# osmr/pytorchcv

Measured on AMD Instinct MI355X. Metric: images/sec @224x224 (resnet50 bs=256/GPU), higher is better.
Workload: dtype bf16; 1 GPU; resnet50_bs256; per_gpu_batch=256, global_batch=256, input=fp32 NCHW 224x224 resident in HBM, parallelism=batch-sharded replicas x1, launcher_choice=timed at capture on this GPU

## Files before the change

include/pcv_amd.h:

```cpp
#ifndef PCV_AMD_H
#define PCV_AMD_H

#include <stddef.h>
#include <stdint.h>

#ifdef __cplusplus
extern "C" {
#endif

#define PCV_ABI_VERSION 5

typedef struct pcv_ctx pcv_ctx;

typedef enum pcv_status {
    PCV_OK = 0,
    PCV_ERR_INVALID = -1,
    PCV_ERR_HIP = -2,
    PCV_ERR_NO_DEVICE = -3,
    PCV_ERR_TOO_LARGE = -4
} pcv_status;

typedef enum pcv_dtype { PCV_F32 = 0, PCV_BF16 = 1, PCV_F16 = 2 } pcv_dtype;

typedef enum pcv_act {
// ... 30 lines not shown
int pcv_fp16_guard_begin(pcv_ctx* ctx, unsigned* slot, void* stream);
int pcv_fp16_guard_end(pcv_ctx* ctx, const unsigned* slot, float* y, long count, void* stream);
int pcv_fp16_overflow_count(pcv_ctx* ctx, unsigned* count, void* stream);

int pcv_nchw_to_nhwc(pcv_ctx* ctx, const float* x, void* y, int N, int C, int H, int W,
                     int cpitch, int wpitch, int dtype, void* stream);
int pcv_nhwc_to_nchw(pcv_ctx* ctx, const void* x, float* y, int N, int C, int H, int W, int cpitch, int dtype,
                     void* stream);

int pcv_preprocess_u8(pcv_ctx* ctx, const unsigned char* x, void* y, int N, int Hs, int Ws, int C, int top, int left,
                      int H, int W, int wpitch, const float* mean, const float* inv_std, int dtype, void* stream);

int pcv_conv_packed_bytes(const pcv_conv_desc* d, size_t* bytes);
int pcv_conv_pack(pcv_ctx* ctx, const pcv_conv_desc* d, const float* w, void* packed, void* stream);
int pcv_dwconv_packed_bytes(const pcv_conv_desc* d, size_t* bytes);
int pcv_dwconv_pack(pcv_ctx* ctx, const pcv_conv_desc* d, const float* w, void* packed, void* stream);
int pcv_bn_fold(pcv_ctx* ctx, int C, const float* gamma, const float* beta, const float* mean, const float* var,
                float eps, const float* conv_bias, float* scale, float* shift, void* stream);

int pcv_conv2d_fused(pcv_ctx* ctx, const pcv_conv_desc* d, const void* x, const void* packed,
                     const float* scale, const float* shift, const void* residual, void* y, void* stream);

int pcv_conv2d_gated_fused(pcv_ctx* ctx, const pcv_conv_desc* d, const void* x, const void* packed, const float* scale,
                           const float* shift, const float* gate, const void* residual, void* y, void* stream);
int pcv_fc_f32(pcv_ctx* ctx, const float* in, const float* w, const float* b, float* out, int N, int K, int J, int act,
               void* stream);
int pcv_conv2d_maxpool_supported(const pcv_conv_desc* d, int k, int s, int p, int ceil_mode);
int pcv_conv2d_maxpool_fused(pcv_ctx* ctx, const pcv_conv_desc* d, const void* x, const void* packed, const float* scale,
                             const float* shift, void* y, int k, int s, int p, int ceil_mode, void* stream);

int pcv_conv2d_nchw_stem_supported(const pcv_conv_desc* d, int pool);
int pcv_conv2d_nchw_stem_fused(pcv_ctx* ctx, const pcv_conv_desc* d, const float* x_nchw, const void* packed, const float* scale,
                               const float* shift, void* y, int pool, void* stream);
int pcv_dwconv2d_fused(pcv_ctx* ctx, const pcv_conv_desc* d, const void* x, const void* packed,
                       const float* scale, const float* shift, const void* residual, void* y, void* stream);
int pcv_maxpool2d(pcv_ctx* ctx, const void* x, void* y, int N, int H, int W, int C, int k, int s, int p,
                  int ceil_mode, int dtype, void* stream);
int pcv_channel_slice(pcv_ctx* ctx, const void* x, void* y, long rows, int C, int offset, int x_cpitch, int y_cpitch,
                      int dtype, void* stream);
int pcv_channel_interleave2(pcv_ctx* ctx, const void* a, const void* b, void* y, long rows, int Ch, int a_cpitch,
                            int b_cpitch, int y_cpitch, int dtype, void* stream);
int pcv_channel_concat(pcv_ctx* ctx, const void* x, void* y, long rows, int C, int x_cpitch, int y_cpitch, int y_offset,
                       int dtype, void* stream);
int pcv_interpolate(pcv_ctx* ctx, const void* x, void* y, int N, int H, int W, int C, int Ho, int Wo, int bilinear,
                    int align_corners, int dtype, void* stream);
int pcv_avgpool2d(pcv_ctx* ctx, const void* x, void* y, int N, int H, int W, int C, int k, int s,
                  int dtype, int out_dtype, void* stream);
int pcv_global_avgpool(pcv_ctx* ctx, const void* x, void* y, int N, int HW, int C, int dtype, int out_dtype,
                       void* stream);
int pcv_gemm_bias(pcv_ctx* ctx, const void* x, const void* packed, const float* bias, void* y,
                  int N, int Cin, int Cout, int dtype, int out_dtype, void* stream);
int pcv_se_squeeze(pcv_ctx* ctx, const void* x, float* mean, int N, int HW, int C, int dtype, void* stream);
int pcv_se_excite(pcv_ctx* ctx, const float* mean, const float* w1, const float* b1, const float* w2,
                  const float* b2, float* mid, float* gate, int N, int C, int M, int mid_act, int out_act,
                  void* stream);
int pcv_se_scale(pcv_ctx* ctx, const void* x, const float* gate, const void* residual, void* y,
                 int N, int HW, int C, int post_act, int dtype, void* stream);

int pcv_splat_squeeze(pcv_ctx* ctx, const void* x, float* s, int N, int HW, int C, int radix, int dtype, void* stream);
int pcv_splat_excite(pcv_ctx* ctx, const float* s, const float* w1, const float* b1, const float* w2, const float* b2, float* mid,
                     float* logits, float* att, int N, int C, int M, int radix, int groups, void* stream);
int pcv_splat_combine(pcv_ctx* ctx, const void* x, const float* att, const void* residual, void* y, int N, int HW, int C, int radix,
                      int post_act, int dtype, void* stream);
int pcv_avgpool2d_pad(pcv_ctx* ctx, const void* x, void* y, int N, int H, int W, int C, int k, int s, int p, int ceil_mode,
                      int count_include_pad, int dtype, int out_dtype, void* stream);

int pcv_conv1x1_pair_supported(const pcv_conv_desc* d1, const pcv_conv_desc* d2);
int pcv_conv1x1_pair_fused(pcv_ctx* ctx, const pcv_conv_desc* d1, const pcv_conv_desc* d2, const void* x,
                           const void* packed1, const float* scale1, const float* shift1, const void* residual, void* y1,
                           const void* packed2, const float* scale2, const float* shift2, void* y2, void* stream);

int pcv_conv1x1_pair_gated_supported(const pcv_conv_desc* d1, const pcv_conv_desc* d2);
int pcv_conv1x1_pair_gated_fused(pcv_ctx* ctx, const pcv_conv_desc* d1, const pcv_conv_desc* d2, const void* x,
                                 const void* packed1, const float* scale1, const float* shift1, const float* gate,
                                 const void* residual, void* y1, const void* packed2, const float* scale2, const float* shift2,
                                 void* y2, void* stream);

int pcv_conv1x1_pair_idconv_supported(const pcv_conv_desc* d_id, const pcv_conv_desc* d1, const pcv_conv_desc* d2);
int pcv_conv1x1_pair_idconv_fused(pcv_ctx* ctx, const pcv_conv_desc* d_id, const pcv_conv_desc* d1, const pcv_conv_desc* d2,
                                  const void* x0, const void* packed_id, const float* scale_id, const float* shift_id,
                                  const void* x, const void* packed1, const float* scale1, const float* shift1, void* y1,
                                  const void* packed2, const float* scale2, const float* shift2, void* y2, void* stream);

int pcv_mbconv_supported(const pcv_conv_desc* d_exp, const pcv_conv_desc* d_dw, const pcv_conv_desc* d_proj);
int pcv_mbconv_fused(pcv_ctx* ctx, const pcv_conv_desc* d_exp, const pcv_conv_desc* d_dw, const pcv_conv_desc* d_proj,
                     const void* x, const void* packed_exp, const float* scale_e, const float* shift_e,
                     const void* packed_dw, const float* scale_d, const float* shift_d, const void* packed_proj,
                     const float* scale_p, const float* shift_p, const void* residual, void* y, void* stream);

int pcv_bn_act(pcv_ctx* ctx, const void* x, const float* scale, const float* shift, void* y, long rows, int C,
               int x_cpitch, int act, int dtype, void* stream);

int pcv_rccl_available(void);
int pcv_rccl_broadcast(pcv_ctx* ctx, void* comm, void* const* bufs, const size_t* bytes, int count, int root, void* stream);
int pcv_rccl_allgather(pcv_ctx* ctx, void* comm, const void* send, void* recv, size_t bytes_per_rank, void* stream);

#ifdef __cplusplus
}
#endif
#endif
```

pytorchcv_amd/_lib.py:

```python

__all__ = ['lib', 'ctx_for', 'check', 'ConvDesc', 'LIB_PATH', 'PcvError', 'PCV_ERR_TOO_LARGE']

import os
import ctypes
import threading

LIB_PATH = os.path.join(os.path.dirname(os.path.abspath(__file__)), "csrc", "libpcv_amd.so")
PCV_ERR_TOO_LARGE = -4

_c = ctypes
_VP = ctypes.c_void_p
_I = ctypes.c_int


class PcvError(RuntimeError):
    def __init__(self, code, msg):
        super(PcvError, self).__init__("pcv_amd error {}: {}".format(code, msg))
        self.code = code


PCV_ABI_VERSION = 5


class ConvDesc(ctypes.Structure):
    _fields_ = [(n, ctypes.c_int32) for n in (
        "struct_size", "N", "H", "W", "Cin", "Cout", "kh", "kw", "stride_h", "stride_w", "pad_t", "pad_l", "pad_b", "pad_r",
        "dil_h", "dil_w", "groups", "act", "post_act", "has_residual", "dtype", "out_dtype", "x_cpitch", "x_wpitch",
        "y_cpitch")]


    def __init__(self, *args, **kw):
        super(ConvDesc, self).__init__(*args, **kw)
        self.struct_size = ctypes.sizeof(ConvDesc)


_SIGS = {
    "pcv_abi_version": (_I, []),
    "pcv_conv_desc_size": (ctypes.c_size_t, []),
    "pcv_create": (_I, [ctypes.POINTER(_VP), _I]),
    "pcv_destroy": (_I, [_VP]),
    "pcv_last_error": (ctypes.c_char_p, [_VP]),
    "pcv_set_tuning": (_I, [_VP, ctypes.c_char_p, _I]),
    "pcv_fp16_guard_begin": (_I, [_VP, _VP, _VP]),
    "pcv_fp16_guard_end": (_I, [_VP, _VP, _VP, ctypes.c_long, _VP]),
    "pcv_fp16_overflow_count": (_I, [_VP, ctypes.POINTER(ctypes.c_uint), _VP]),
    "pcv_rccl_available": (_I, []),
    "pcv_rccl_broadcast": (_I, [_VP, _VP, ctypes.POINTER(_VP), ctypes.POINTER(ctypes.c_size_t), _I, _I, _VP]),
    "pcv_rccl_allgather": (_I, [_VP, _VP, _VP, _VP, ctypes.c_size_t, _VP]),
    "pcv_nchw_to_nhwc": (_I, [_VP, _VP, _VP, _I, _I, _I, _I, _I, _I, _I, _VP]),
    "pcv_nhwc_to_nchw": (_I, [_VP, _VP, _VP, _I, _I, _I, _I, _I, _I, _VP]),
    "pcv_preprocess_u8": (_I, [_VP, _VP, _VP, _I, _I, _I, _I, _I, _I, _I, _I, _I, _VP, _VP, _I, _VP]),
    "pcv_conv_packed_bytes": (_I, [ctypes.POINTER(ConvDesc), ctypes.POINTER(ctypes.c_size_t)]),
    "pcv_conv_pack": (_I, [_VP, ctypes.POINTER(ConvDesc), _VP, _VP, _VP]),
    "pcv_dwconv_packed_bytes": (_I, [ctypes.POINTER(ConvDesc), ctypes.POINTER(ctypes.c_size_t)]),
    "pcv_dwconv_pack": (_I, [_VP, ctypes.POINTER(ConvDesc), _VP, _VP, _VP]),
    "pcv_bn_fold": (_I, [_VP, _I, _VP, _VP, _VP, _VP, ctypes.c_float, _VP, _VP, _VP, _VP]),
    "pcv_conv2d_fused": (_I, [_VP, ctypes.POINTER(ConvDesc), _VP, _VP, _VP, _VP, _VP, _VP, _VP]),
    "pcv_dwconv2d_fused": (_I, [_VP, ctypes.POINTER(ConvDesc), _VP, _VP, _VP, _VP, _VP, _VP, _VP]),
    "pcv_maxpool2d": (_I, [_VP, _VP, _VP, _I, _I, _I, _I, _I, _I, _I, _I, _I, _VP]),
    "pcv_channel_slice": (_I, [_VP, _VP, _VP, ctypes.c_long, _I, _I, _I, _I, _I, _VP]),
    "pcv_channel_interleave2": (_I, [_VP, _VP, _VP, _VP, ctypes.c_long, _I, _I, _I, _I, _I, _VP]),
    "pcv_channel_concat": (_I, [_VP, _VP, _VP, ctypes.c_long, _I, _I, _I, _I, _I, _VP]),
    "pcv_interpolate": (_I, [_VP, _VP, _VP, _I, _I, _I, _I, _I, _I, _I, _I, _I, _VP]),
    "pcv_avgpool2d": (_I, [_VP, _VP, _VP, _I, _I, _I, _I, _I, _I, _I, _I, _VP]),
    "pcv_global_avgpool": (_I, [_VP, _VP, _VP, _I, _I, _I, _I, _I, _VP]),
    "pcv_gemm_bias": (_I, [_VP, _VP, _VP, _VP, _VP, _I, _I, _I, _I, _I, _VP]),
    "pcv_se_squeeze": (_I, [_VP, _VP, _VP, _I, _I, _I, _I, _VP]),
    "pcv_se_excite": (_I, [_VP, _VP, _VP, _VP, _VP, _VP, _VP, _VP, _I, _I, _I, _I, _I, _VP]),
    "pcv_conv2d_gated_fused": (_I, [_VP, ctypes.POINTER(ConvDesc), _VP, _VP, _VP, _VP, _VP, _VP, _VP, _VP]),
    "pcv_fc_f32": (_I, [_VP, _VP, _VP, _VP, _VP, _I, _I, _I, _I, _VP]),
    "pcv_conv2d_maxpool_supported": (_I, [ctypes.POINTER(ConvDesc), _I, _I, _I, _I]),
    "pcv_conv2d_maxpool_fused": (_I, [_VP, ctypes.POINTER(ConvDesc), _VP, _VP, _VP, _VP, _VP, _I, _I, _I, _I, _VP]),
    "pcv_conv2d_nchw_stem_supported": (_I, [ctypes.POINTER(ConvDesc), _I]),
    "pcv_conv2d_nchw_stem_fused": (_I, [_VP, ctypes.POINTER(ConvDesc), _VP, _VP, _VP, _VP, _VP, _I, _VP]),
    "pcv_conv1x1_pair_supported": (_I, [ctypes.POINTER(ConvDesc), ctypes.POINTER(ConvDesc)]),
    "pcv_conv1x1_pair_fused": (_I, [_VP, ctypes.POINTER(ConvDesc), ctypes.POINTER(ConvDesc), _VP, _VP, _VP, _VP, _VP, _VP, _VP,
                                    _VP, _VP, _VP, _VP]),
    "pcv_conv1x1_pair_gated_supported": (_I, [ctypes.POINTER(ConvDesc), ctypes.POINTER(ConvDesc)]),
    "pcv_conv1x1_pair_gated_fused": (_I, [_VP, ctypes.POINTER(ConvDesc), ctypes.POINTER(ConvDesc), _VP, _VP, _VP, _VP, _VP, _VP, _VP,
                                          _VP, _VP, _VP, _VP, _VP]),
    "pcv_conv1x1_pair_idconv_supported": (_I, [ctypes.POINTER(ConvDesc), ctypes.POINTER(ConvDesc), ctypes.POINTER(ConvDesc)]),
    "pcv_conv1x1_pair_idconv_fused": (_I, [_VP, ctypes.POINTER(ConvDesc), ctypes.POINTER(ConvDesc), ctypes.POINTER(ConvDesc),
                                           _VP, _VP, _VP, _VP, _VP, _VP, _VP, _VP, _VP, _VP, _VP, _VP, _VP, _VP]),
    "pcv_mbconv_supported": (_I, [ctypes.POINTER(ConvDesc), ctypes.POINTER(ConvDesc), ctypes.POINTER(ConvDesc)]),
    "pcv_mbconv_fused": (_I, [_VP, ctypes.POINTER(ConvDesc), ctypes.POINTER(ConvDesc), ctypes.POINTER(ConvDesc), _VP, _VP, _VP, _VP,
                              _VP, _VP, _VP, _VP, _VP, _VP, _VP, _VP, _VP]),
    "pcv_bn_act": (_I, [_VP, _VP, _VP, _VP, _VP, ctypes.c_long, _I, _I, _I, _I, _VP]),
    "pcv_se_scale": (_I, [_VP, _VP, _VP, _VP, _VP, _I, _I, _I, _I, _I, _VP]),
    "pcv_splat_squeeze": (_I, [_VP, _VP, _VP, _I, _I, _I, _I, _I, _VP]),
    "pcv_splat_excite": (_I, [_VP, _VP, _VP, _VP, _VP, _VP, _VP, _VP, _VP, _I, _I, _I, _I, _I, _VP]),
    "pcv_splat_combine": (_I, [_VP, _VP, _VP, _VP, _VP, _I, _I, _I, _I, _I, _I, _VP]),
    "pcv_avgpool2d_pad": (_I, [_VP, _VP, _VP, _I, _I, _I, _I, _I, _I, _I, _I, _I, _I, _I, _VP]),
}

_lib = None
_ctxs = {}
_lock = threading.RLock()


def lib():
    global _lib
    if _lib is None:
        with _lock:
            if _lib is None:
                if not os.path.exists(LIB_PATH):
                    raise RuntimeError(
                        "pytorchcv_amd: HIP extension {} is missing - build it with `python -c 'import __graft_entry__ as g; "
                        "g.build()'` or `make -C pytorchcv_amd/csrc`. There is no CPU fallback.".format(LIB_PATH))
                L = ctypes.CDLL(LIB_PATH)
                for name, (res, args) in _SIGS.items():
                    fn = getattr(L, name)
                    fn.restype = res
                    fn.argtypes = args
                if L.pcv_abi_version() != PCV_ABI_VERSION or L.pcv_conv_desc_size() != ctypes.sizeof(ConvDesc):
                    raise RuntimeError("pytorchcv_amd: {} has ABI version {} / a {}-byte pcv_conv_desc, this binding expects "
                                       "version {} / {} bytes - rebuild the library".format(
                                           LIB_PATH, L.pcv_abi_version(), L.pcv_conv_desc_size(), PCV_ABI_VERSION,
                                           ctypes.sizeof(ConvDesc)))
                _lib = L
    return _lib


def exported_symbols():
    return sorted(_SIGS.keys())


def ctx_for(device_index: int):
    c = _ctxs.get(device_index)
    if c is None:
        with _lock:
            c = _ctxs.get(device_index)
            if c is None:
                L = lib()
                h = _VP()
                rc = L.pcv_create(ctypes.byref(h), int(device_index))
                if rc != 0:
                    raise PcvError(rc, (L.pcv_last_error(None) or b"").decode())
                c = h
                _ctxs[device_index] = c
    return c


def check(rc: int, ctx):
    if rc != 0:
        raise PcvError(rc, (lib().pcv_last_error(ctx) or b"").decode())
```

pytorchcv_amd/csrc/pcv_api.hip:

```cpp
#include <hip/hip_runtime.h>
#include <string>
#include <vector>
#include <cstring>
#include <algorithm>
#include <cstdio>
#include <cstdlib>
#include <dlfcn.h>
#include "pcv_common.hpp"
#include "igemm_inst.hpp"
#include "d3q_inst.hpp"
#include "d3w_inst.hpp"
#include "d3c_conv.hpp"
#include "d3k_conv.hpp"
#include "d3i_conv.hpp"
#include "d1i_conv.hpp"
#include "p1r_conv.hpp"
#include "stem_conv.hpp"
#include "pair1x1.hpp"
#include "wpair1x1.hpp"
#include "gconv3x3.hpp"
#include "gconv3x3r.hpp"
#include "mbconv.hpp"
#include "mbw_inst.hpp"
#include "mbr_inst.hpp"
MBW_SHAPES(MBW_DECLARE, PCV_BF16)
MBW_SHAPES(MBW_DECLARE, PCV_F16)
MBW2_SHAPES(MBW2_DECLARE, PCV_BF16)
MBW2_SHAPES(MBW2_DECLARE, PCV_F16)
MBW3_SHAPES(MBW3_DECLARE, PCV_BF16)
MBW3_SHAPES(MBW3_DECLARE, PCV_F16)
MBR_SHAPES(MBR_DECLARE, PCV_BF16)
MBR_SHAPES(MBR_DECLARE, PCV_F16)
#include "dwconv.hpp"
#include "aux_kernels.hpp"
#include "head_gemm.hpp"


IGEMM_INSTANCES(IGEMM_DECLARE, PCV_BF16)
IGEMM_INSTANCES(IGEMM_DECLARE, PCV_F16)
IGEMM_INSTANCES_SAMETYPE(IGEMM_DECLARE, PCV_F32)
D3Q_SHAPES(D3Q_DECLARE, PCV_BF16)
D3Q_SHAPES(D3Q_DECLARE, PCV_F16)
D3Q1_SHAPES(D3Q1_DECLARE, PCV_BF16)
D3Q1_SHAPES(D3Q1_DECLARE, PCV_F16)
D3W_SHAPES(D3W_DECLARE, PCV_BF16)
D3W_SHAPES(D3W_DECLARE, PCV_F16)
D3WT_SHAPES(D3WT_DECLARE, PCV_BF16)
D3WT_SHAPES(D3WT_DECLARE, PCV_F16)
extern template __global__ void d3c_kernel<PCV_BF16>(const D3Params);
extern template __global__ void d3c_kernel<PCV_F16>(const D3Params);
extern template __global__ void d3k_kernel<PCV_BF16>(const D3Params);
extern template __global__ void d3k_kernel<PCV_F16>(const D3Params);
extern template __global__ void d3i_kernel<PCV_BF16, 256>(const D3Params);
extern template __global__ void d3i_kernel<PCV_F16, 256>(const D3Params);
extern template __global__ void d3i_kernel<PCV_BF16, 512>(const D3Params);
extern template __global__ void d3i_kernel<PCV_F16, 512>(const D3Params);
extern template __global__ void d1i_kernel<PCV_BF16, 1024>(const D3Params);
extern template __global__ void d1i_kernel<PCV_F16, 1024>(const D3Params);
extern template __global__ void d1i_kernel<PCV_BF16, 2048>(const D3Params);
extern template __global__ void d1i_kernel<PCV_F16, 2048>(const D3Params);
#define P1R_DECLARE(CW, CIN)                                                       \
    extern template __global__ void p1r_kernel<PCV_BF16, CW, CIN>(const D3Params); \
    extern template __global__ void p1r_kernel<PCV_F16, CW, CIN>(const D3Params);
P1R_DECLARE(64, 256)
P1R_DECLARE(32, 512)
P1R_DECLARE(32, 256)

struct pcv_ctx {
    int device = 0;
    std::string err;
    int num_cu = 256;
    int persist_mode = 1;
    int force_tile = -1;
    int use_wstat = 1;
    int use_mbr = 1;
    int use_mbw = 1;
    int use_gconvr = 1;
    int use_d1x1 = -1;
    int use_head = 1;
    int use_stem32 = 1;
    int use_d3x3 = -1;
    unsigned long long dbg_ptr = 0;
    int use_p1r = -1;
    int use_d3k = -1;
    int use_d3i = -1;
    int use_d1i = -1;
    int use_d3c = -1;
    int use_d3w = -1;
    int dbg_flags = 0;
    int dw_flags = 0;
    int dw_th = 0;
    int max_blocks = 0;
    int pair_pb = 2;
    int persist_max_nk = 4;
    uint32_t* ovf = nullptr;
};

static thread_local std::string g_create_err;

static int fail(pcv_ctx* ctx, int code, const std::string& msg) {
    if (ctx) ctx->err = msg; else g_create_err = msg;
    return code;
}
#define HIP_TRY(ctx, expr)                                                                          \
    do {                                                                                            \
        hipError_t e__ = (expr);                                                                    \
        if (e__ != hipSuccess)                                                                      \
            return fail(ctx, PCV_ERR_HIP, std::string(#expr) + ": " + hipGetErrorString(e__));      \
    } while (0)

struct DeviceGuard {
    int prev = -1;
    bool switched = false;
    explicit DeviceGuard(int want) {
        if (hipGetDevice(&prev) == hipSuccess && prev != want) switched = hipSetDevice(want) == hipSuccess;
    }
    ~DeviceGuard() {
        if (switched) (void)hipSetDevice(prev);
    }
};

static inline int round_up(int v, int m) { return (v + m - 1) / m * m; }
static inline long long block_slots(const pcv_ctx* ctx, int per_cu) {
    const long long n = (long long)ctx->num_cu * per_cu;
    return (ctx->max_blocks > 0 && ctx->max_blocks < n) ? ctx->max_blocks : n;
}
static inline int esize(int dt) { return dt == PCV_F32 ? 4 : 2; }
static inline bool dtype_ok(int dt) { return dt == PCV_F32 || dt == PCV_BF16 || dt == PCV_F16; }
static inline bool aligned16(const void* p) { return (reinterpret_cast<uintptr_t>(p) & 15u) == 0; }

struct ConvPlan {
    bool stem = false;
    bool conv3 = false;
    int ES = 2, CE = 8;
    bool pair = false;
    int Ho = 0, Wo = 0;
    int ngb = 1;
    int Cg_in = 0, Cg_out = 0;
    int cin_blk = 0, cout_blk = 0;
    int nR = 1, nQ = 1;
    int dy[IGEMM_MAX_TAPS], dx[IGEMM_MAX_TAPS];
    int nchunks = 0, nk = 0, Kpad = 0;
    int wrows = 0;
    size_t ktab_bytes = 0, w_bytes = 0, total_bytes = 0;
    int gconv_kt = 5;
    bool gconv = false;
    bool d3i = false;
    bool d1i = false;
    size_t d3i_off = 0;
    size_t gconv_off = 0;
    std::vector<uint32_t> ktab;
    std::vector<uint32_t> ksrc;
};

static const char* kStaleDesc = "pcv_conv_desc.struct_size does not match this library (stale binding: compare pcv_conv_desc_size() / PCV_ABI_VERSION)";
static inline bool desc_stale(const pcv_conv_desc& d) { return d.struct_size != (int32_t)sizeof(pcv_conv_desc); }

static const char* plan_conv(const pcv_conv_desc& d, ConvPlan& P, bool tables) {
    if (desc_stale(d)) return kStaleDesc;
    if (!dtype_ok(d.dtype) || !dtype_ok(d.out_dtype)) return "unknown dtype";
    if (d.out_dtype != d.dtype && d.out_dtype != PCV_F32) return "out_dtype must equal dtype or be fp32";
    if (d.Cin <= 0 || d.Cout <= 0 || d.kh <= 0 || d.kw <= 0 || d.groups <= 0) return "non-positive conv dimension";
    constexpr int kMaxChannels = 1 << 20, kMaxExtent = 1 << 24, kMaxGeom = 1 << 12;
    if (d.Cin > kMaxChannels || d.Cout > kMaxChannels || d.groups > kMaxChannels) return "channel count out of range (> 2^20)";
    if (d.N < 0 || d.H < 0 || d.W < 0 || d.N > kMaxExtent || d.H > kMaxExtent || d.W > kMaxExtent) return "N / H / W out of range (> 2^24)";
    if (d.stride_h > kMaxGeom || d.stride_w > kMaxGeom || d.dil_h > kMaxGeom || d.dil_w > kMaxGeom) return "stride / dilation out of range";
    if (d.pad_t < 0 || d.pad_l < 0 || d.pad_b < 0 || d.pad_r < 0 || d.pad_t > kMaxGeom || d.pad_l > kMaxGeom || d.pad_b > kMaxGeom ||
        d.pad_r > kMaxGeom)
        return "padding out of range";
    if (d.x_cpitch < 0 || d.x_cpitch > 8 * kMaxChannels || d.x_wpitch < 0 || d.x_wpitch > 2 * kMaxExtent || d.y_cpitch < 0 ||
        d.y_cpitch > 8 * kMaxChannels)
        return "pitch out of range";
    if (d.kh >= IGEMM_MAX_TAPS || d.kw >= IGEMM_MAX_TAPS) return "kernel size > 15 unsupported";
    if (d.stride_h <= 0 || d.stride_w <= 0 || d.dil_h <= 0 || d.dil_w <= 0) return "non-positive stride/dilation";
    if (d.Cin % d.groups || d.Cout % d.groups) return "channels not divisible by groups";
    P.ES = esize(d.dtype);
    P.CE = 16 / P.ES;
    P.Cg_in = d.Cin / d.groups;
    P.Cg_out = d.Cout / d.groups;
    const int cpitch = d.x_cpitch > 0 ? d.x_cpitch : d.Cin;
    if (cpitch < d.Cin) return "x_cpitch < Cin";
    P.pair = (d.groups == 1 && cpitch == 4 && P.ES == 2);
    if (!P.pair && cpitch % P.CE != 0) return "x_cpitch must be a multiple of 16 bytes (or 4 for a padded 16-bit stem)";

    int gpb = 1;
    if (d.groups > 1) {
        while (gpb < d.groups && ((gpb * P.Cg_out) % 8 != 0 || (gpb * P.Cg_in) % P.CE != 0 || gpb * P.Cg_out < 32)) ++gpb;
        while (gpb < d.groups && d.groups % gpb != 0) ++gpb;
        if (d.groups % gpb != 0 || (gpb * P.Cg_out) % 8 != 0 || (gpb * P.Cg_in) % P.CE != 0)
            return "unsupported group shape (channels per group block not 16-byte aligned)";
    }
    P.ngb = d.groups / gpb;
    P.cin_blk = gpb * P.Cg_in;
    P.cout_blk = gpb * P.Cg_out;
    if (d.groups == 1) P.cin_blk = d.Cin;
    P.wrows = round_up(P.cout_blk, 32);

    P.conv3 = d.groups == 1 && d.kh == 3 && d.kw == 3 && d.stride_h == 1 && d.stride_w == 1 && d.dil_h == 1 && d.dil_w == 1 &&
              d.pad_t == 1 && d.pad_l == 1 && d.pad_b == 1 && d.pad_r == 1 && d.Cin % (8 * P.CE) == 0 && cpitch == d.Cin &&
              (d.x_wpitch <= 0 || d.x_wpitch == d.W) && d.out_dtype == d.dtype && d.Cout % 8 == 0;

    P.stem = P.pair && d.stride_h == 2 && d.stride_w == 2 && d.dil_h == 1 && d.Cout <= 64 && d.Cout % 8 == 0 && d.kh <= 7 &&
             d.kw + (d.pad_l & 1) <= 8 && d.out_dtype == d.dtype;

    if (P.pair) {
        if (d.stride_w % 2 != 0 || d.dil_w != 1) return "padded 4-channel stem needs even stride_w and dilation 1";
        const int wp = d.x_wpitch > 0 ? d.x_wpitch : d.W;
        if (wp % 2 != 0) return "padded 4-channel stem needs an even x_wpitch";
        const int dxs = -(d.pad_l & 1);
        P.nQ = (d.kw - dxs + 1) / 2;
        P.nR = d.kh;
        if (P.nQ >= IGEMM_MAX_TAPS) return "stem too wide";
        for (int r = 0; r < P.nR; ++r) P.dy[r] = r * d.dil_h;
        for (int q = 0; q < P.nQ; ++q) P.dx[q] = dxs + 2 * q;
        P.nchunks = P.nR * P.nQ;
    } else {
        P.nR = d.kh;
        P.nQ = d.kw;
        for (int r = 0; r < P.nR; ++r) P.dy[r] = r * d.dil_h;
        for (int q = 0; q < P.nQ; ++q) P.dx[q] = q * d.dil_w;
        const int cchunks = (P.cin_blk + P.CE - 1) / P.CE;
        if (d.groups == 1 && cchunks * P.CE > cpitch) return "x_cpitch too small for the channel chunks";
        P.nchunks = P.nR * P.nQ * cchunks;
    }
    for (int i = P.nR; i < IGEMM_MAX_TAPS; ++i) P.dy[i] = 0;
    for (int i = P.nQ; i < IGEMM_MAX_TAPS; ++i) P.dx[i] = 0;
    P.nk = (P.nchunks + 7) / 8;
    P.Kpad = P.nk * 8 * P.CE;
    P.ktab_bytes = (size_t)round_up(P.nk * 8 * 8, 256);
    P.w_bytes = (size_t)P.ngb * P.wrows * P.Kpad * P.ES;
    P.total_bytes = P.ktab_bytes + P.w_bytes;
    static const bool gconv_on = !(std::getenv("PCV_AMD_GCONV") && std::atoi(std::getenv("PCV_AMD_GCONV")) == 0);
    P.gconv = gconv_on && d.groups > 1 && d.kh == 3 && d.kw == 3 && d.stride_h == d.stride_w && (d.stride_h == 1 || d.stride_h == 2) &&
              d.dil_h == 1 && d.dil_w == 1 &&
              d.pad_t == 1 && d.pad_l == 1 && d.pad_b == 1 && d.pad_r == 1 && d.Cin == d.Cout && d.Cin % 64 == 0 && P.ES == 2 &&
              (P.Cg_in == 4 || P.Cg_in == 8 || P.Cg_in == 16 || P.Cg_in == 32) && d.out_dtype == d.dtype;
    if (P.gconv) {
        P.gconv_kt = P.Cg_in == 32 ? 9 : 5;
        P.gconv_off = (P.total_bytes + 15) / 16 * 16;
        P.total_bytes = P.gconv_off + (size_t)(d.Cin / 16) * P.gconv_kt * 16 * 32 * P.ES;
    }
    P.d3i = P.conv3 && P.ES == 2 && (d.Cin == 256 || d.Cin == 512) && d.Cout % D3ICfg::CW == 0 && d.out_dtype == d.dtype &&
            P.wrows >= d.Cout && P.Kpad == 9 * d.Cin;
    if (P.d3i) {
        P.d3i_off = (P.total_bytes + 15) / 16 * 16;
        P.total_bytes = P.d3i_off + (size_t)(d.Cout / D3ICfg::CW) * (d.Cin == 256 ? D3ICfgT<256>::WBYTES : D3ICfgT<512>::WBYTES);
    }
    P.d1i = !P.conv3 && !P.pair && !P.stem && P.ES == 2 && d.kh == 1 && d.kw == 1 && d.groups == 1 && d.stride_h == 1 && d.stride_w == 1 &&
            d.pad_t == 0 && d.pad_l == 0 && d.pad_b == 0 && d.pad_r == 0 && (d.Cin == 1024 || d.Cin == 2048) &&
            d.Cout % 64 == 0 && d.out_dtype == d.dtype && P.wrows >= d.Cout && P.Kpad == d.Cin && P.ngb == 1;
    if (P.d1i) {
        P.d3i_off = (P.total_bytes + 15) / 16 * 16;
        P.total_bytes = P.d3i_off + (size_t)(d.Cout / 64) * (size_t)(d.Cin / 32) * 4096;
    }
    if (P.w_bytes >= 0x80000000ull) return "packed weights exceed 2 GiB";

    if (P.stem) {
        P.ktab_bytes = 0;
        P.w_bytes = (size_t)d.kh * 64 * 32 * P.ES;
        P.total_bytes = P.w_bytes;
    }
    P.Ho = (d.H + d.pad_t + d.pad_b - d.dil_h * (d.kh - 1) - 1) / d.stride_h + 1;
    P.Wo = (d.W + d.pad_l + d.pad_r - d.dil_w * (d.kw - 1) - 1) / d.stride_w + 1;

    if (tables) {
        P.ktab.assign((size_t)P.nk * 8 * 2, 0);
        P.ksrc.assign((size_t)P.Kpad, 0xFFFFFFFFu);
        const int khkw = d.kh * d.kw;
        (void)khkw;
        int j = 0;
        auto put = [&](int c0, int r, int q, int dyv, int dxv) {
            P.ktab[2 * j] = (uint32_t)c0 | ((uint32_t)r << 16) | ((uint32_t)q << 20);
            P.ktab[2 * j + 1] = ((uint32_t)dyv & 0xFFFFu) | (((uint32_t)dxv & 0xFFFFu) << 16);
            ++j;
        };
        if (P.pair) {
            for (int r = 0; r < P.nR; ++r)
                for (int q = 0; q < P.nQ; ++q) {
                    for (int e = 0; e < 8; ++e) {
                        const int pix = e >> 2, c = e & 3;
                        const int tap = P.dx[q] + pix;
                        if (tap >= 0 && tap < d.kw && c < d.Cin)
                            P.ksrc[(size_t)j * 8 + e] = (uint32_t)c | ((uint32_t)(r * d.kw + tap) << 16);
                    }
                    put(0, r, q, P.dy[r], P.dx[q]);
                }
        } else if (P.conv3) {
            const int slices = d.Cin / (8 * P.CE);
            for (int r = 0; r < 3; ++r)
                for (int cs = 0; cs < slices; ++cs)
                    for (int q = 0; q < 3; ++q)
                        for (int cc = cs * 8; cc < cs * 8 + 8; ++cc) {
                            for (int e = 0; e < P.CE; ++e)
                                P.ksrc[(size_t)j * P.CE + e] = (uint32_t)(cc * P.CE + e) | ((uint32_t)(r * 3 + q) << 16);
                            put(cc * P.CE, r, q, P.dy[r], P.dx[q]);
                        }
        } else {
            const int cchunks = (P.cin_blk + P.CE - 1) / P.CE;
            for (int r = 0; r < P.nR; ++r)
                for (int q = 0; q < P.nQ; ++q)
                    for (int cc = 0; cc < cchunks; ++cc) {
                        for (int e = 0; e < P.CE; ++e) {
                            const int c = cc * P.CE + e;
                            if (c < P.cin_blk)
                                P.ksrc[(size_t)j * P.CE + e] = (uint32_t)c | ((uint32_t)(r * d.kw + q) << 16);
                        }
                        put(cc * P.CE, r, q, P.dy[r], P.dx[q]);
                    }
        }
        while (j < P.nk * 8) put(0, 15, 0, 0, 0);
    }
    return nullptr;
}

enum TileCfg { TILE_C32 = 0, TILE_C64 = 1, TILE_C128 = 2, TILE_C256 = 3, TILE_C64S = 4, TILE_C128S = 5, TILE_COUNT = 6 };
struct TileInfo { int BM, BP, threads, lds; };
static const TileInfo kTiles[TILE_COUNT] = {
    {32, 256, 256, 2 * (32 + 256) * 128},
    {64, 256, 256, 2 * (64 + 256) * 128},
    {128, 128, 256, 2 * (128 + 128) * 128},
    {256, 64, 256, 2 * (256 + 64) * 128},
    {64, 128, 256, 2 * (64 + 128) * 128},
    {128, 64, 256, 2 * (128 + 64) * 128},
};
typedef void (*igemm_fn)(const IgemmParams);

template <int DT, int KHW> static igemm_fn igemm_for_tile(int tile) {
    switch (tile) {
        case TILE_C32: return igemm_conv_kernel<DT, DT, 2, 4, 1, 4, false, KHW>;
        case TILE_C64: return igemm_conv_kernel<DT, DT, 4, 4, 1, 4, false, KHW>;
        case TILE_C128: return igemm_conv_kernel<DT, DT, 4, 4, 2, 2, false, KHW>;
        case TILE_C256: return igemm_conv_kernel<DT, DT, 4, 4, 4, 1, false, KHW>;
        case TILE_C64S: if constexpr (KHW == 1) return igemm_conv_kernel<DT, DT, 4, 2, 1, 4, false, 1>; else return nullptr;
        case TILE_C128S: if constexpr (KHW == 1) return igemm_conv_kernel<DT, DT, 4, 2, 2, 2, false, 1>; else return nullptr;
// ... 52 lines not shown

typedef void (*gconv_fn)(const GConvParams);
struct GConvLaunch { gconv_fn fn; int lds; };
static GConvLaunch pick_gconv(int dt, int W) {
    const bool bf = dt == PCV_BF16;
    if (W + 1 <= 16) return GConvLaunch{bf ? gconv3x3_kernel<PCV_BF16, 16> : gconv3x3_kernel<PCV_F16, 16>, GConvCfg<16>::LDS};
    if (W + 1 <= 32) return GConvLaunch{bf ? gconv3x3_kernel<PCV_BF16, 32> : gconv3x3_kernel<PCV_F16, 32>, GConvCfg<32>::LDS};
    return GConvLaunch{bf ? gconv3x3_kernel<PCV_BF16, 64> : gconv3x3_kernel<PCV_F16, 64>, GConvCfg<64>::LDS};
}
typedef void (*gconvr_fn)(const GConvRParams);
static gconvr_fn pick_gconvr(int dt, int stride, int kt) {
    const bool bf = dt == PCV_BF16;
    if (stride == 2) {
        if (kt == 9) return bf ? gconv3x3r_kernel<PCV_BF16, 2, 9> : gconv3x3r_kernel<PCV_F16, 2, 9>;
        return bf ? gconv3x3r_kernel<PCV_BF16, 2, 5> : gconv3x3r_kernel<PCV_F16, 2, 5>;
    }
    return bf ? gconv3x3r_kernel<PCV_BF16, 1, 9> : gconv3x3r_kernel<PCV_F16, 1, 9>;
}
struct GConvRPlan { int R, XH, xl, win; };
static bool plan_gconvr(int stride, int H, int W, int Ho, int Wo, GConvRPlan& g) {
    if (stride == 2 && ((H | W) & 1)) return false;
    if (Wo > 64 || Ho <= 0) return false;
    for (int R = 64 / Wo; R >= 1; --R) {
        const int win = stride == 2 ? (2 * R + 1) * W + 2 : (R + 2) * W + 2;
        const int XH = stride == 2 ? ((win + 1) / 2 + 7) / 8 * 8 : 0;
        const int rows = ((stride == 2 ? 2 * XH : win) + 31) / 32 * 32;
        const int lds = 2 * rows * 128;
        if (lds * 2 <= 160 * 1024 || (R == 1 && lds <= 160 * 1024)) {
            g.R = R; g.XH = XH; g.xl = rows / 32; g.win = win;
            return true;
        }
    }
    return false;
}
static int enable_gconvr(pcv_ctx* ctx) {
    for (int dt = PCV_BF16; dt <= PCV_F16; ++dt)
        for (int s = 1; s <= 2; ++s)
            for (int kt = 5; kt <= 9; kt += 4)
                HIP_TRY(ctx, hipFuncSetAttribute(reinterpret_cast<const void*>(pick_gconvr(dt, s, kt)),
                                                 hipFuncAttributeMaxDynamicSharedMemorySize, 160 * 1024));
    return PCV_OK;
}
static int g_gconv_blocks_per_cu[3] = {2, 2, 2};
static int enable_gconv(pcv_ctx* ctx) {
    const int widths[3] = {15, 31, 63};
    for (int i = 0; i < 3; ++i)
        for (int dt = PCV_BF16; dt <= PCV_F16; ++dt) {
            const GConvLaunch L = pick_gconv(dt, widths[i]);
            HIP_TRY(ctx, hipFuncSetAttribute(reinterpret_cast<const void*>(L.fn), hipFuncAttributeMaxDynamicSharedMemorySize, L.lds));
            int nb = 0;
            HIP_TRY(ctx, hipOccupancyMaxActiveBlocksPerMultiprocessor(&nb, reinterpret_cast<const void*>(L.fn), 256, L.lds));
            g_gconv_blocks_per_cu[i] = nb < 1 ? 1 : nb;
        }
    return PCV_OK;
}
struct D3Shape { int BM, BP, lds; const void* fn[2]; };
#define D3Q_ROW(DT, WC, WP, CBW, PBW, KS)                                                                    \
    {D3Cfg<WC, WP, CBW, PBW, KS>::BM, D3Cfg<WC, WP, CBW, PBW, KS>::BP, D3Cfg<WC, WP, CBW, PBW, KS>::LDS,     \
     {reinterpret_cast<const void*>(d3q_kernel<PCV_BF16, WC, WP, CBW, PBW, KS>),                             \
      reinterpret_cast<const void*>(d3q_kernel<PCV_F16, WC, WP, CBW, PBW, KS>)}},
static const D3Shape kD3[] = {D3Q_SHAPES(D3Q_ROW, 0)};
static const int kD3Count = (int)(sizeof(kD3) / sizeof(kD3[0]));
#define D3Q1_ROW(DT, WC, WP, CBW, PBW, KS)                                                                                     \
    {D3Cfg<WC, WP, CBW, PBW, KS, true>::BM, D3Cfg<WC, WP, CBW, PBW, KS, true>::BP, D3Cfg<WC, WP, CBW, PBW, KS, true>::LDS,      \
     {reinterpret_cast<const void*>(d3q_kernel<PCV_BF16, WC, WP, CBW, PBW, KS, true>),                                        \
      reinterpret_cast<const void*>(d3q_kernel<PCV_F16, WC, WP, CBW, PBW, KS, true>)}},
static const D3Shape kD1[] = {D3Q1_SHAPES(D3Q1_ROW, 0)};
static const int kD1Count = (int)(sizeof(kD1) / sizeof(kD1[0]));
#define D3W_ROW(DT, WC, WP, CBW, PBW, KS, NSA)                                                                                   \
    {D3WCfg<WC, WP, CBW, PBW, KS, NSA>::BM, D3WCfg<WC, WP, CBW, PBW, KS, NSA>::BP, D3WCfg<WC, WP, CBW, PBW, KS, NSA>::LDS,       \
     {reinterpret_cast<const void*>(d3w_kernel<PCV_BF16, WC, WP, CBW, PBW, KS, NSA>),                                           \
      reinterpret_cast<const void*>(d3w_kernel<PCV_F16, WC, WP, CBW, PBW, KS, NSA>)}},
#define D3WT_ROW(DT, WC, WP, CBW, PBW, KS, NSA, TRIM)                                                                                               \
    {D3WCfg<WC, WP, CBW, PBW, KS, NSA, TRIM>::BM, D3WCfg<WC, WP, CBW, PBW, KS, NSA, TRIM>::BP, D3WCfg<WC, WP, CBW, PBW, KS, NSA, TRIM>::LDS,       \
     {reinterpret_cast<const void*>(d3w_kernel<PCV_BF16, WC, WP, CBW, PBW, KS, NSA, TRIM>),                                                       \
      reinterpret_cast<const void*>(d3w_kernel<PCV_F16, WC, WP, CBW, PBW, KS, NSA, TRIM>)}},
static const D3Shape kD3W[] = {D3W_SHAPES(D3W_ROW, 0) D3WT_SHAPES(D3WT_ROW, 0)};
static const int kD3WCount = (int)(sizeof(kD3W) / sizeof(kD3W[0]));
static const void* kD3C[2] = {reinterpret_cast<const void*>(d3c_kernel<PCV_BF16>), reinterpret_cast<const void*>(d3c_kernel<PCV_F16>)};
static const void* kD3I[2][2] = {{reinterpret_cast<const void*>(d3i_kernel<PCV_BF16, 256>), reinterpret_cast<const void*>(d3i_kernel<PCV_F16, 256>)},
                                 {reinterpret_cast<const void*>(d3i_kernel<PCV_BF16, 512>), reinterpret_cast<const void*>(d3i_kernel<PCV_F16, 512>)}};
static const void* kD1I[2][2] = {{reinterpret_cast<const void*>(d1i_kernel<PCV_BF16, 1024>), reinterpret_cast<const void*>(d1i_kernel<PCV_F16, 1024>)},
                                 {reinterpret_cast<const void*>(d1i_kernel<PCV_BF16, 2048>), reinterpret_cast<const void*>(d1i_kernel<PCV_F16, 2048>)}};
static const void* kD3K[2] = {reinterpret_cast<const void*>(d3k_kernel<PCV_BF16>), reinterpret_cast<const void*>(d3k_kernel<PCV_F16>)};
#define P1R_ROW(CW, CIN)                                                                   \
    {P1RCfg<CW, CIN>::BM, P1RCfg<CW, CIN>::BP, P1RCfg<CW, CIN>::LDS,                       \
     {reinterpret_cast<const void*>(p1r_kernel<PCV_BF16, CW, CIN>), reinterpret_cast<const void*>(p1r_kernel<PCV_F16, CW, CIN>)}}
static const D3Shape kP1R[3] = {P1R_ROW(64, 256), P1R_ROW(32, 512), P1R_ROW(32, 256)};
static int enable_d3x3(pcv_ctx* ctx) {
    for (int i = 0; i < 3; ++i)
        for (int t = 0; t < 2; ++t) HIP_TRY(ctx, hipFuncSetAttribute(kP1R[i].fn[t], hipFuncAttributeMaxDynamicSharedMemorySize, kP1R[i].lds));
    for (int t = 0; t < 2; ++t) HIP_TRY(ctx, hipFuncSetAttribute(kD3C[t], hipFuncAttributeMaxDynamicSharedMemorySize, D3CCfg::LDS));
    for (int t = 0; t < 2; ++t) HIP_TRY(ctx, hipFuncSetAttribute(kD3K[t], hipFuncAttributeMaxDynamicSharedMemorySize, D3KCfg::LDS));
    for (int i = 0; i < 2; ++i)
        for (int t = 0; t < 2; ++t) HIP_TRY(ctx, hipFuncSetAttribute(kD1I[i][t], hipFuncAttributeMaxDynamicSharedMemorySize, D1ICfgT<1024>::LDS));
    for (int t = 0; t < 2; ++t) HIP_TRY(ctx, hipFuncSetAttribute(kD3I[0][t], hipFuncAttributeMaxDynamicSharedMemorySize, D3ICfgT<256>::LDS));
    for (int t = 0; t < 2; ++t) HIP_TRY(ctx, hipFuncSetAttribute(kD3I[1][t], hipFuncAttributeMaxDynamicSharedMemorySize, D3ICfgT<512>::LDS));
    for (int i = 0; i < kD3WCount; ++i)
        for (int t = 0; t < 2; ++t)
            HIP_TRY(ctx, hipFuncSetAttribute(kD3W[i].fn[t], hipFuncAttributeMaxDynamicSharedMemorySize, kD3W[i].lds));

    for (int i = 0; i < kD3Count; ++i)
        for (int t = 0; t < 2; ++t)
            HIP_TRY(ctx, hipFuncSetAttribute(kD3[i].fn[t], hipFuncAttributeMaxDynamicSharedMemorySize, kD3[i].lds));
    for (int i = 0; i < kD1Count; ++i)
        for (int t = 0; t < 2; ++t)
            HIP_TRY(ctx, hipFuncSetAttribute(kD1[i].fn[t], hipFuncAttributeMaxDynamicSharedMemorySize, kD1[i].lds));
    return PCV_OK;
}
static int pick_d1x1(long long M, int Cout, int Cin, long long slots) {
    if (Cin < 256 || Cout < 128) return -1;
    const int shape = Cout % 256 == 0 ? 1 : 0;
    const long long tiles = (long long)((Cout + kD1[shape].BM - 1) / kD1[shape].BM) * ((M + kD1[shape].BP - 1) / kD1[shape].BP);
    return tiles * 2 >= slots ? shape : -1;
}
static int pick_d3x3(long long M, int Cout, int nk, long long slots) {
    (void)nk;
    const int wide = Cout <= 64 ? 2 : 1, narrow = Cout <= 64 ? 5 : 4;
    auto tiles = [&](int i) { return ((Cout + kD3[i].BM - 1) / kD3[i].BM) * ((M + kD3[i].BP - 1) / kD3[i].BP); };
    if (Cout % 256 == 0 && tiles(0) * 2 >= slots) return 0;
    if (tiles(wide) * 2 >= slots) return wide;
    if (tiles(narrow) * 4 >= slots) return narrow;
    return -1;
}
static int pick_d3w(long long M, int Cout, long long slots) {
    const int shape = Cout % 256 == 0 ? 1 : (Cout % 128 == 0 ? 2 : -1);
    if (shape < 0) return -1;
    const long long tiles = (long long)(Cout / kD3W[shape].BM) * ((M + kD3W[shape].BP - 1) / kD3W[shape].BP);
    return tiles * 4 >= slots * 3 ? shape : -1;
}

static const int kStemLds = 7 * 64 * 64 + 2 * 768 * 16 + 3 * 2 * 64 * 16;
static int g_stem_blocks_per_cu[2];
static int enable_stem(pcv_ctx* ctx) {
    const void* fns[2] = {reinterpret_cast<const void*>(stem_conv_kernel<PCV_BF16, false>),
                          reinterpret_cast<const void*>(stem_conv_kernel<PCV_F16, false>)};
    const void* pooled[2] = {reinterpret_cast<const void*>(stem_conv_kernel<PCV_BF16, true>),
                             reinterpret_cast<const void*>(stem_conv_kernel<PCV_F16, true>)};
    for (int i = 0; i < 2; ++i) HIP_TRY(ctx, hipFuncSetAttribute(pooled[i], hipFuncAttributeMaxDynamicSharedMemorySize, kStemLds));
    const void* from_nchw[4] = {reinterpret_cast<const void*>(stem_conv_kernel<PCV_BF16, false, true>),
                                reinterpret_cast<const void*>(stem_conv_kernel<PCV_F16, false, true>),
                                reinterpret_cast<const void*>(stem_conv_kernel<PCV_BF16, true, true>),
                                reinterpret_cast<const void*>(stem_conv_kernel<PCV_F16, true, true>)};
    for (int i = 0; i < 4; ++i)
        HIP_TRY(ctx, hipFuncSetAttribute(from_nchw[i], hipFuncAttributeMaxDynamicSharedMemorySize, kStemLds + kStemStageBytes));
    const void* narrow[4] = {reinterpret_cast<const void*>(stem_conv_kernel<PCV_BF16, false, false, 2>),
                             reinterpret_cast<const void*>(stem_conv_kernel<PCV_F16, false, false, 2>),
                             reinterpret_cast<const void*>(stem_conv_kernel<PCV_BF16, false, true, 2>),
                             reinterpret_cast<const void*>(stem_conv_kernel<PCV_F16, false, true, 2>)};
    for (int i = 0; i < 4; ++i)
        HIP_TRY(ctx, hipFuncSetAttribute(narrow[i], hipFuncAttributeMaxDynamicSharedMemorySize, kStemLds + (i >= 2 ? kStemStageBytes : 0)));
    for (int i = 0; i < 2; ++i) {
        HIP_TRY(ctx, hipFuncSetAttribute(fns[i], hipFuncAttributeMaxDynamicSharedMemorySize, kStemLds));
        int nb = 0;
        HIP_TRY(ctx, hipOccupancyMaxActiveBlocksPerMultiprocessor(&nb, fns[i], 256, kStemLds));
        g_stem_blocks_per_cu[i] = nb < 1 ? 1 : nb;
    }
    return PCV_OK;
}

static int pair_lds(int pb, bool idc = false) { return (idc ? 6 : 3) * 16 * pb * 64 * 2 + 16 * 1024 * pb + (idc ? 4096 : 0); }
static int g_pair_idc_blocks_per_cu = 1;
static int g_pair_blocks_per_cu[2] = {1, 1};
static int g_wpair_mask = 3;
static int g_wpair_blocks_per_cu[4] = {1, 1, 1, 1};
struct WPairLaunch { const void* fn; int threads, lds, tileP; bool gate_in_lds; };
template <int CM, int C1> static WPairLaunch wpair_launch_for(int dt, bool gated) {
    typedef WPairCfg<CM, C1> G;
    const void* fn;
    if (gated) fn = dt == PCV_BF16 ? reinterpret_cast<const void*>(wpair1x1_kernel<PCV_BF16, CM, C1, true>)
                                   : reinterpret_cast<const void*>(wpair1x1_kernel<PCV_F16, CM, C1, true>);
    else fn = dt == PCV_BF16 ? reinterpret_cast<const void*>(wpair1x1_kernel<PCV_BF16, CM, C1, false>)
                             : reinterpret_cast<const void*>(wpair1x1_kernel<PCV_F16, CM, C1, false>);
    return WPairLaunch{fn, 64 * G::NW, gated ? G::LDS_GATED : G::LDS, G::P, gated && G::GATE_LDS};
}
static WPairLaunch wpair_launch(int cfg, int dt, bool gated = false) {
    switch (cfg) {
        case 0: return wpair_launch_for<128, 512>(dt, gated);
        case 1: return wpair_launch_for<256, 1024>(dt, gated);
        case 2: return wpair_launch_for<128, 256>(dt, gated);
        default: return wpair_launch_for<256, 512>(dt, gated);
    }
}
static int wpair_cfg(int cm, int c1) {
    if (cm == 128 && c1 == 512) return 0;
    if (cm == 256 && c1 == 1024) return 1;
    if (cm == 128 && c1 == 256) return 2;
    if (cm == 256 && c1 == 512) return 3;
    return -1;
}
static int enable_pair(pcv_ctx* ctx) {
    const void* fns[4] = {reinterpret_cast<const void*>(pair1x1_kernel<PCV_BF16, 4>),
                          reinterpret_cast<const void*>(pair1x1_kernel<PCV_F16, 4>),
                          reinterpret_cast<const void*>(pair1x1_kernel<PCV_BF16, 2>),
                          reinterpret_cast<const void*>(pair1x1_kernel<PCV_F16, 2>)};
    for (int i = 0; i < 4; ++i) {
        const int lds = pair_lds(i < 2 ? 4 : 2);
        HIP_TRY(ctx, hipFuncSetAttribute(fns[i], hipFuncAttributeMaxDynamicSharedMemorySize, lds));
        int nb = 0;
        HIP_TRY(ctx, hipOccupancyMaxActiveBlocksPerMultiprocessor(&nb, fns[i], 256, lds));
        g_pair_blocks_per_cu[i / 2] = nb < 1 ? 1 : nb;
    }
    const void* gated[2] = {reinterpret_cast<const void*>(pair1x1_kernel<PCV_BF16, 2, false, true>),
                            reinterpret_cast<const void*>(pair1x1_kernel<PCV_F16, 2, false, true>)};
    for (int i = 0; i < 2; ++i) HIP_TRY(ctx, hipFuncSetAttribute(gated[i], hipFuncAttributeMaxDynamicSharedMemorySize, pair_lds(2)));
    const void* idc[2] = {reinterpret_cast<const void*>(pair1x1_kernel<PCV_BF16, 2, true>),
                          reinterpret_cast<const void*>(pair1x1_kernel<PCV_F16, 2, true>)};
    for (int i = 0; i < 2; ++i) {
        HIP_TRY(ctx, hipFuncSetAttribute(idc[i], hipFuncAttributeMaxDynamicSharedMemorySize, pair_lds(2, true)));
        int nb = 0;
        HIP_TRY(ctx, hipOccupancyMaxActiveBlocksPerMultiprocessor(&nb, idc[i], 256, pair_lds(2, true)));
        g_pair_idc_blocks_per_cu = nb < 1 ? 1 : nb;
    }
    for (int cfg = 0; cfg < 4; ++cfg)
        for (int dt = PCV_BF16; dt <= PCV_F16; ++dt) {
            const WPairLaunch L = wpair_launch(cfg, dt);
            HIP_TRY(ctx, hipFuncSetAttribute(L.fn, hipFuncAttributeMaxDynamicSharedMemorySize, L.lds));
            HIP_TRY(ctx, hipFuncSetAttribute(wpair_launch(cfg, dt, true).fn, hipFuncAttributeMaxDynamicSharedMemorySize,
                                             wpair_launch(cfg, dt, true).lds));
            int nb = 0;
            HIP_TRY(ctx, hipOccupancyMaxActiveBlocksPerMultiprocessor(&nb, L.fn, L.threads, L.lds));
            g_wpair_blocks_per_cu[cfg] = nb < 1 ? 1 : nb;
        }
    return PCV_OK;
}
static const char* pair_unsupported(const pcv_conv_desc& a, const pcv_conv_desc& b) {
    if (desc_stale(a) || desc_stale(b)) return kStaleDesc;
    auto plain1x1 = [](const pcv_conv_desc& d) {
        return d.kh == 1 && d.kw == 1 && d.stride_h == 1 && d.stride_w == 1 && d.pad_t == 0 && d.pad_l == 0 && d.pad_b == 0 &&
               d.pad_r == 0 && d.groups == 1 && d.dil_h == 1 && d.dil_w == 1 && d.out_dtype == d.dtype &&
               (d.x_cpitch == 0 || d.x_cpitch == d.Cin) && (d.x_wpitch == 0 || d.x_wpitch == d.W) &&
               (d.y_cpitch == 0 || d.y_cpitch == d.Cout);
    };
    if (!plain1x1(a) || !plain1x1(b)) return "both convolutions must be plain 1x1 stride 1";
    if (a.dtype != b.dtype || (a.dtype != PCV_BF16 && a.dtype != PCV_F16)) return "16-bit storage only";
    if (a.N != b.N || a.H != b.H || a.W != b.W || a.Cout != b.Cin) return "shapes do not chain";
    const bool narrow = a.Cin == 64 && a.Cout == 256 && b.Cout == 64;
    const bool wide = ((a.Cin == 128 && (g_wpair_mask & 1)) || (a.Cin == 256 && (g_wpair_mask & 2))) &&
                      wpair_cfg(a.Cin, a.Cout) >= 0 && b.Cout == a.Cin;
    if (!narrow && !wide) return "only 64 -> 256 -> 64, 128 -> 512|256 -> 128 and 256 -> 1024|512 -> 256 are instantiated";
    if (!a.has_residual || b.has_residual || b.post_act != PCV_ACT_NONE) return "first conv must carry the residual, second must not";
    if ((long)a.N * a.H * a.W * a.Cout * 2 >= (1L << 31)) return "tensor exceeds the 2 GiB window";
    return nullptr;
}

typedef void (*mbconv_fn)(const MbParams);
// ... 118 lines not shown
    else if (d.stride_h == 1) dwconv5_kernel<DT, 1, FAST><<<grid, 256, 0, s>>>(p);
    else dwconv5_kernel<DT, 2, FAST><<<grid, 256, 0, s>>>(p);
}
template <int DT> static void launch_dw(const pcv_conv_desc& d, const DwParams& p, unsigned grid, hipStream_t s) {
    if (d.act <= PCV_ACT_RELU6 && d.post_act <= PCV_ACT_RELU6) launch_dw2<DT, true>(d, p, grid, s);
    else launch_dw2<DT, false>(d, p, grid, s);
}
template <int DT> static void launch_mean(const void* x, void* y, int N, int HW, int C, int ot, hipStream_t s, int radix = 1) {
    dim3 grid((unsigned)N, (unsigned)((C / 8 + 511) / 512));
    if (ot == PCV_F32) spatial_mean_kernel<DT, PCV_F32><<<grid, 512, 0, s>>>(x, y, HW, C, radix);
    else spatial_mean_kernel<DT, DT><<<grid, 512, 0, s>>>(x, y, HW, C, radix);
}
template <int DT> static void launch_avg(const void* x, void* y, int N, int H, int W, int C, int Ho, int Wo, int k, int s,
                                         int ot, hipStream_t st, int pad = 0, int count_pad = 1, uint32_t* ovf = nullptr) {
    const long total = (long)N * Ho * Wo * (C / 8);
    const unsigned grid = (unsigned)((total + 255) / 256);
    if (ot == PCV_F32) avgpool_kernel<DT, PCV_F32><<<grid, 256, 0, st>>>(x, y, N, H, W, C, Ho, Wo, k, s, pad, count_pad, ovf);
    else avgpool_kernel<DT, DT><<<grid, 256, 0, st>>>(x, y, N, H, W, C, Ho, Wo, k, s, pad, count_pad, ovf);
}


extern "C" {

int pcv_abi_version(void) { return PCV_ABI_VERSION; }

size_t pcv_conv_desc_size(void) { return sizeof(pcv_conv_desc); }

const char* pcv_last_error(const pcv_ctx* ctx) { return ctx ? ctx->err.c_str() : g_create_err.c_str(); }

int pcv_create(pcv_ctx** out, int device) {
    if (out == nullptr) return fail(nullptr, PCV_ERR_INVALID, "pcv_create: out is NULL");
    *out = nullptr;
    int count = 0;
    if (hipGetDeviceCount(&count) != hipSuccess || count <= 0)
        return fail(nullptr, PCV_ERR_NO_DEVICE, "pcv_create: no HIP device visible");
    if (device < 0 || device >= count) return fail(nullptr, PCV_ERR_INVALID, "pcv_create: bad device index");
    hipDeviceProp_t prop;
    HIP_TRY(nullptr, hipGetDeviceProperties(&prop, device));
    if (std::strncmp(prop.gcnArchName, "gfx950", 6) != 0)
        return fail(nullptr, PCV_ERR_NO_DEVICE,
                    std::string("pcv_create: device is ") + prop.gcnArchName + ", this library is built for gfx950 only");
    int prev = 0;
    HIP_TRY(nullptr, hipGetDevice(&prev));
    HIP_TRY(nullptr, hipSetDevice(device));
    pcv_ctx* ctx = new (std::nothrow) pcv_ctx();
    if (ctx == nullptr) return fail(nullptr, PCV_ERR_INVALID, "pcv_create: out of host memory");
    ctx->device = device;
    ctx->num_cu = prop.multiProcessorCount;
    if (const char* e = std::getenv("PCV_AMD_PERSIST")) ctx->persist_mode = std::atoi(e);
    if (const char* e = std::getenv("PCV_AMD_PERSIST_NK")) ctx->persist_max_nk = std::atoi(e);
    int rc = enable_big_lds(ctx);
    if (rc == PCV_OK) rc = enable_d3x3(ctx);
    if (rc == PCV_OK) rc = enable_gconv(ctx);
    if (rc == PCV_OK) rc = enable_gconvr(ctx);
    if (rc == PCV_OK) rc = enable_stem(ctx);
    if (rc == PCV_OK) rc = enable_pair(ctx);
    if (rc == PCV_OK) rc = enable_mbconv(ctx);
    if (rc == PCV_OK) {
        hipError_t e = hipMalloc(reinterpret_cast<void**>(&ctx->ovf), 256);
        if (e == hipSuccess) e = hipMemset(ctx->ovf, 0, 256);
        if (e != hipSuccess) rc = fail(ctx, PCV_ERR_HIP, std::string("pcv_create: overflow counter: ") + hipGetErrorString(e));
    }
    if (rc != PCV_OK) {
        g_create_err = ctx->err;
        if (ctx->ovf) (void)hipFree(ctx->ovf);
        delete ctx;
        (void)hipSetDevice(prev);
        return rc;
    }
    (void)hipSetDevice(prev);
    *out = ctx;
    return PCV_OK;
}

int pcv_set_tuning(pcv_ctx* ctx, const char* key, int value) {
    if (!ctx || !key) return PCV_ERR_INVALID;
    const std::string k(key);
    if (k == "persist") ctx->persist_mode = value;
    else if (k == "persist_nk") ctx->persist_max_nk = value;
    else if (k == "tile") ctx->force_tile = value;
    else if (k == "pair_pb") ctx->pair_pb = value;
    else if (k == "mbw_wide") g_mbw_wide = value;
    else if (k == "wpair") g_wpair_mask = value;
    else if (k == "max_blocks") ctx->max_blocks = value;
    else if (k == "d3x3") ctx->use_d3x3 = value;
    else if (k == "d3w") ctx->use_d3w = value;
    else if (k == "d3c") ctx->use_d3c = value;
    else if (k == "d3k") ctx->use_d3k = value;
    else if (k == "d3i") ctx->use_d3i = value;
    else if (k == "d1i") ctx->use_d1i = value;
    else if (k == "p1r") ctx->use_p1r = value;
    else if (k == "head") ctx->use_head = value;
    else if (k == "stem32") ctx->use_stem32 = value;
    else if (k == "d1x1") ctx->use_d1x1 = value;
    else if (k == "gconvr") ctx->use_gconvr = value;
    else if (k == "mbw") ctx->use_mbw = value;
    else if (k == "mbr") ctx->use_mbr = value;
    else if (k == "mbr_xl") g_mbr_xl = value;
    else if (k == "dbg") {
#ifdef PCV_DBG_FLAGS
        ctx->dbg_flags = value;
#else
        if (value != 0)
            return fail(ctx, PCV_ERR_INVALID, "pcv_set_tuning: \"dbg\" (timing experiments that produce wrong results) needs a -DPCV_DBG_FLAGS build");
#endif
    }
    else if (k == "dw_th") ctx->dw_th = value;
    else if (k == "dw_flags") ctx->dw_flags = value;
    else if (k == "dbg_lo") ctx->dbg_ptr = (ctx->dbg_ptr & 0xFFFFFFFF00000000ull) | (unsigned)value;
    else if (k == "dbg_hi") ctx->dbg_ptr = (ctx->dbg_ptr & 0xFFFFFFFFull) | ((unsigned long long)(unsigned)value << 32);
    else if (k == "wstat") ctx->use_wstat = value;
    else return fail(ctx, PCV_ERR_INVALID, "pcv_set_tuning: unknown key " + k);
    return PCV_OK;
}

int pcv_destroy(pcv_ctx* ctx) {
    if (ctx && ctx->ovf) {
        DeviceGuard device_guard(ctx->device);
        (void)hipFree(ctx->ovf);
    }
    delete ctx;
    return PCV_OK;
}

int pcv_fp16_guard_begin(pcv_ctx* ctx, unsigned* slot, void* stream) {
    if (!ctx) return PCV_ERR_INVALID;
    DeviceGuard device_guard(ctx->device);
    if (!slot) return fail(ctx, PCV_ERR_INVALID, "pcv_fp16_guard_begin: slot is NULL");
    f16_guard_begin_kernel<<<1, 1, 0, (hipStream_t)stream>>>(ctx->ovf, slot);
    HIP_TRY(ctx, hipGetLastError());
    return PCV_OK;
}

int pcv_fp16_guard_end(pcv_ctx* ctx, const unsigned* slot, float* y, long count, void* stream) {
    if (!ctx) return PCV_ERR_INVALID;
    DeviceGuard device_guard(ctx->device);
    if (!slot || !y || count <= 0) return fail(ctx, PCV_ERR_INVALID, "pcv_fp16_guard_end: bad argument");
    const unsigned grid = (unsigned)std::min<long>((count + 255) / 256, 1024);
    f16_guard_end_kernel<<<grid, 256, 0, (hipStream_t)stream>>>(ctx->ovf, slot, y, count);
    HIP_TRY(ctx, hipGetLastError());
    return PCV_OK;
}

extern "C++" {
namespace {
typedef int (*nccl_group_fn)(void);
typedef int (*nccl_bcast_fn)(const void*, void*, size_t, int, int, void*, hipStream_t);
typedef int (*nccl_gather_fn)(const void*, void*, size_t, int, void*, hipStream_t);
typedef const char* (*nccl_err_fn)(int);
struct RcclApi {
    nccl_group_fn group_start = nullptr, group_end = nullptr;
    nccl_bcast_fn broadcast = nullptr;
    nccl_gather_fn allgather = nullptr;
    nccl_err_fn error_string = nullptr;
    bool ok = false;
};
const RcclApi& rccl_api() {
    static const RcclApi api = [] {
        RcclApi a;
        void* h = dlopen("librccl.so.1", RTLD_NOW | RTLD_NOLOAD);
        if (!h) h = dlopen("librccl.so.1", RTLD_NOW);
        if (!h) h = dlopen("librccl.so", RTLD_NOW);
        if (!h) return a;
        a.group_start = reinterpret_cast<nccl_group_fn>(dlsym(h, "ncclGroupStart"));
        a.group_end = reinterpret_cast<nccl_group_fn>(dlsym(h, "ncclGroupEnd"));
        a.broadcast = reinterpret_cast<nccl_bcast_fn>(dlsym(h, "ncclBroadcast"));
// ... 66 lines not shown
    else if (dtype == PCV_F16) nchw_to_nhwc_kernel<PCV_F16><<<grid, 256, 0, s>>>(x, y, N, C, H, W, cpitch, wpitch, ctx->ovf);
    else nchw_to_nhwc_kernel<PCV_F32><<<grid, 256, 0, s>>>(x, y, N, C, H, W, cpitch, wpitch, ctx->ovf);
    HIP_TRY(ctx, hipGetLastError());
    return PCV_OK;
}

int pcv_nhwc_to_nchw(pcv_ctx* ctx, const void* x, float* y, int N, int C, int H, int W, int cpitch, int dtype, void* stream) {
    if (!ctx) return PCV_ERR_INVALID;
    DeviceGuard device_guard(ctx->device);
    if (cpitch <= 0) cpitch = C;
    if (!x || !y || N <= 0 || C <= 0 || H <= 0 || W <= 0 || cpitch < C || !dtype_ok(dtype))
        return fail(ctx, PCV_ERR_INVALID, "pcv_nhwc_to_nchw: bad argument");
    const long total = (long)N * C * H * W;
    const unsigned grid = (unsigned)((total + 255) / 256);
    hipStream_t s = (hipStream_t)stream;
    if (dtype == PCV_BF16) nhwc_to_nchw_kernel<PCV_BF16><<<grid, 256, 0, s>>>(x, y, N, C, H, W, cpitch);
    else if (dtype == PCV_F16) nhwc_to_nchw_kernel<PCV_F16><<<grid, 256, 0, s>>>(x, y, N, C, H, W, cpitch);
    else nhwc_to_nchw_kernel<PCV_F32><<<grid, 256, 0, s>>>(x, y, N, C, H, W, cpitch);
    HIP_TRY(ctx, hipGetLastError());
    return PCV_OK;
}

int pcv_conv_packed_bytes(const pcv_conv_desc* d, size_t* bytes) {
    if (!d || !bytes) return PCV_ERR_INVALID;
    ConvPlan P;
    if (plan_conv(*d, P, false) != nullptr) return PCV_ERR_INVALID;
    *bytes = P.total_bytes;
    return PCV_OK;
}

int pcv_conv_pack(pcv_ctx* ctx, const pcv_conv_desc* d, const float* w, void* packed, void* stream) {
    if (!ctx) return PCV_ERR_INVALID;
    DeviceGuard device_guard(ctx->device);
    if (!d || !w || !packed) return fail(ctx, PCV_ERR_INVALID, "pcv_conv_pack: NULL argument");
    if (!aligned16(packed)) return fail(ctx, PCV_ERR_INVALID, "pcv_conv_pack: packed buffer must be 16-byte aligned");
    ConvPlan P;
    const char* why = plan_conv(*d, P, true);
    if (why) return fail(ctx, PCV_ERR_INVALID, std::string("pcv_conv_pack: ") + why);
    hipStream_t s = (hipStream_t)stream;
    if (P.stem) {
        const int total = d->kh * 64 * 32;
        if (d->dtype == PCV_BF16) pack_stem_kernel<PCV_BF16><<<(total + 255) / 256, 256, 0, s>>>(w, packed, d->Cout, d->Cin, d->kh, d->kw, d->pad_l & 1);
        else pack_stem_kernel<PCV_F16><<<(total + 255) / 256, 256, 0, s>>>(w, packed, d->Cout, d->Cin, d->kh, d->kw, d->pad_l & 1);
        HIP_TRY(ctx, hipGetLastError());
        return PCV_OK;
    }
    uint32_t* ksrc_dev = nullptr;
    HIP_TRY(ctx, hipStreamSynchronize(s));
    HIP_TRY(ctx, hipMalloc(reinterpret_cast<void**>(&ksrc_dev), P.ksrc.size() * sizeof(uint32_t)));
    hipError_t e = hipMemcpy(ksrc_dev, P.ksrc.data(), P.ksrc.size() * sizeof(uint32_t), hipMemcpyHostToDevice);
    if (e == hipSuccess) e = hipMemcpy(packed, P.ktab.data(), P.ktab.size() * sizeof(uint32_t), hipMemcpyHostToDevice);
    if (e != hipSuccess) {
        (void)hipFree(ksrc_dev);
        return fail(ctx, PCV_ERR_HIP, std::string("pcv_conv_pack: table upload: ") + hipGetErrorString(e));
    }
    PackParams pp;
    pp.w = w;
    pp.out = static_cast<char*>(packed) + P.ktab_bytes;
    pp.ksrc = ksrc_dev;
    pp.ngb = P.ngb;
    pp.wrows = P.wrows;
    pp.Kpad = P.Kpad;
    pp.cout_blk = P.cout_blk;
    pp.cin_blk = d->groups == 1 ? 0 : P.cin_blk;
    pp.Cg_in = P.Cg_in;
    pp.Cg_out = P.Cg_out;
    pp.khkw = d->kh * d->kw;
    const long total = (long)P.ngb * P.wrows * P.Kpad;
    const unsigned grid = (unsigned)((total + 255) / 256);
    if (d->dtype == PCV_BF16) pack_conv_kernel<PCV_BF16><<<grid, 256, 0, s>>>(pp);
    else if (d->dtype == PCV_F16) pack_conv_kernel<PCV_F16><<<grid, 256, 0, s>>>(pp);
    else pack_conv_kernel<PCV_F32><<<grid, 256, 0, s>>>(pp);
    if (P.gconv) {
        const long gtotal = (long)(d->Cin / 16) * P.gconv_kt * 16 * 32;
        const unsigned ggrid = (unsigned)((gtotal + 255) / 256);
        void* gout = static_cast<char*>(packed) + P.gconv_off;
        const bool bf = d->dtype == PCV_BF16;
        if (P.gconv_kt == 9) {
            if (bf) pack_gconv32_kernel<PCV_BF16><<<ggrid, 256, 0, s>>>(w, gout, d->Cin);
            else pack_gconv32_kernel<PCV_F16><<<ggrid, 256, 0, s>>>(w, gout, d->Cin);
        } else if (bf) pack_gconv_kernel<PCV_BF16><<<ggrid, 256, 0, s>>>(w, gout, d->Cin, P.Cg_in);
        else pack_gconv_kernel<PCV_F16><<<ggrid, 256, 0, s>>>(w, gout, d->Cin, P.Cg_in);
    }
    if (P.d3i || P.d1i) {
        const int total = (int)((P.total_bytes - P.d3i_off) / 16);
        pack_d3i_kernel<<<(unsigned)((total + 255) / 256), 256, 0, s>>>(reinterpret_cast<const u32x4*>(pp.out),
                                                                        reinterpret_cast<u32x4*>(static_cast<char*>(packed) + P.d3i_off), P.Kpad, total);
    }
    e = hipGetLastError();
    if (e == hipSuccess) e = hipStreamSynchronize(s);
    (void)hipFree(ksrc_dev);
    if (e != hipSuccess) return fail(ctx, PCV_ERR_HIP, std::string("pcv_conv_pack: ") + hipGetErrorString(e));
    return PCV_OK;
}

static const char* check_dw(const pcv_conv_desc& d) {
    if (desc_stale(d)) return kStaleDesc;
    if (!dtype_ok(d.dtype) || d.out_dtype != d.dtype) return "depthwise: out_dtype must equal dtype";
    if (d.groups != d.Cin || d.Cin != d.Cout) return "depthwise: needs groups == Cin == Cout";
    if (d.Cin % 8 != 0) return "depthwise: channels must be a multiple of 8";
    if (d.kh != d.kw || (d.kh != 3 && d.kh != 5)) return "depthwise: only 3x3 and 5x5";
    if (d.stride_h != d.stride_w || (d.stride_h != 1 && d.stride_h != 2)) return "depthwise: stride 1 or 2";
    if (d.dil_h != 1 || d.dil_w != 1) return "depthwise: dilation unsupported";
    if (d.x_cpitch > 0 && d.x_cpitch != d.Cin) return "depthwise: padded channel pitch unsupported";
    if (d.x_wpitch > 0 && d.x_wpitch != d.W) return "depthwise: padded row pitch unsupported";
    if (d.y_cpitch > 0 && d.y_cpitch != d.Cout) return "depthwise: y must be dense";
    return nullptr;
}

static size_t dw_taps_bytes(const pcv_conv_desc& d) { return (((size_t)d.kh * d.kw * d.Cin * esize(d.dtype)) + 15) & ~(size_t)15; }
static size_t dw_sparse_bytes(const pcv_conv_desc& d) {
    return (d.kh == 3 && d.dtype != PCV_F32) ? (size_t)((d.Cin + 31) / 32) * 6 * 1024 : 0;
}
int pcv_dwconv_packed_bytes(const pcv_conv_desc* d, size_t* bytes) {
    if (!d || !bytes || check_dw(*d)) return PCV_ERR_INVALID;
    *bytes = dw_taps_bytes(*d) + dw_sparse_bytes(*d);
    return PCV_OK;
}

int pcv_dwconv_pack(pcv_ctx* ctx, const pcv_conv_desc* d, const float* w, void* packed, void* stream) {
    if (!ctx) return PCV_ERR_INVALID;
    DeviceGuard device_guard(ctx->device);
    if (!d || !w || !packed) return fail(ctx, PCV_ERR_INVALID, "pcv_dwconv_pack: NULL argument");
    const char* why = check_dw(*d);
    if (why) return fail(ctx, PCV_ERR_INVALID, std::string("pcv_dwconv_pack: ") + why);
    const int total = d->Cin * d->kh * d->kw;
    const unsigned grid = (unsigned)((total + 255) / 256);
    hipStream_t s = (hipStream_t)stream;
    if (d->dtype == PCV_BF16) pack_dw_kernel<PCV_BF16><<<grid, 256, 0, s>>>(w, packed, d->Cin, d->kh * d->kw);
    else if (d->dtype == PCV_F16) pack_dw_kernel<PCV_F16><<<grid, 256, 0, s>>>(w, packed, d->Cin, d->kh * d->kw);
    else pack_dw_kernel<PCV_F32><<<grid, 256, 0, s>>>(w, packed, d->Cin, d->kh * d->kw);
    if (dw_sparse_bytes(*d) != 0) {
        const int nChunks = (d->Cin + 31) / 32;
        pack_dw_sparse_kernel<<<(unsigned)((nChunks * 6 * 64 + 255) / 256), 256, 0, s>>>(
            static_cast<const uint16_t*>(packed), reinterpret_cast<u32x4*>(static_cast<char*>(packed) + dw_taps_bytes(*d)), d->Cin, nChunks);
    }
    HIP_TRY(ctx, hipGetLastError());
    return PCV_OK;
}

int pcv_bn_fold(pcv_ctx* ctx, int C, const float* gamma, const float* beta, const float* mean, const float* var,
                float eps, const float* conv_bias, float* scale, float* shift, void* stream) {
    if (!ctx) return PCV_ERR_INVALID;
    DeviceGuard device_guard(ctx->device);
    if (C <= 0 || !scale || !shift) return fail(ctx, PCV_ERR_INVALID, "pcv_bn_fold: bad argument");
    const bool any = gamma || beta || mean || var;
    const bool all = gamma && beta && mean && var;
    if (any && !all) return fail(ctx, PCV_ERR_INVALID, "pcv_bn_fold: gamma/beta/mean/var must be all set or all NULL");
    bn_fold_kernel<<<(C + 255) / 256, 256, 0, (hipStream_t)stream>>>(C, gamma, beta, mean, var, eps, conv_bias, scale, shift);
    HIP_TRY(ctx, hipGetLastError());
    return PCV_OK;
}

static int pool_out(int in, int k, int s, int p, int ceil_mode);
static void launch_se_fc(const float* in, const float* w, const float* b, float* out, int N, int K, int J, int act, hipStream_t st);

enum ConvKernel {
    CK_STEM,
    CK_GCONV_ROWS,
    CK_GCONV_FLAT,
    CK_D3I,
    CK_D1I,
    CK_D3K,
    CK_D3C,
    CK_D3W,
    CK_D3Q,
    CK_P1R,
// ... 941 lines not shown
    return PCV_OK;
}

int pcv_channel_slice(pcv_ctx* ctx, const void* x, void* y, long rows, int C, int offset, int x_cpitch, int y_cpitch, int dtype,
                      void* stream) {
    if (!ctx) return PCV_ERR_INVALID;
    DeviceGuard device_guard(ctx->device);
    if (!x || !y || rows <= 0 || C <= 0 || offset < 0 || x_cpitch < offset + C || y_cpitch < C || y_cpitch % 8 != 0 || !dtype_ok(dtype))
        return fail(ctx, PCV_ERR_INVALID, "pcv_channel_slice: bad argument (y_cpitch must be a multiple of 8 and hold C channels)");
    const long total = rows * (y_cpitch / 8);
    const unsigned grid = (unsigned)((total + 255) / 256);
    hipStream_t st = (hipStream_t)stream;
    if (dtype == PCV_BF16) channel_slice_kernel<PCV_BF16><<<grid, 256, 0, st>>>(x, y, rows, C, offset, x_cpitch, y_cpitch);
    else if (dtype == PCV_F16) channel_slice_kernel<PCV_F16><<<grid, 256, 0, st>>>(x, y, rows, C, offset, x_cpitch, y_cpitch);
    else channel_slice_kernel<PCV_F32><<<grid, 256, 0, st>>>(x, y, rows, C, offset, x_cpitch, y_cpitch);
    HIP_TRY(ctx, hipGetLastError());
    return PCV_OK;
}

int pcv_channel_concat(pcv_ctx* ctx, const void* x, void* y, long rows, int C, int x_cpitch, int y_cpitch, int y_offset, int dtype,
                       void* stream) {
    if (!ctx) return PCV_ERR_INVALID;
    DeviceGuard device_guard(ctx->device);
    if (!x || !y || rows <= 0 || C <= 0 || C % 8 != 0 || x_cpitch < C || x_cpitch % 8 != 0 || y_offset < 0 || y_offset % 8 != 0 ||
        y_cpitch < y_offset + C || y_cpitch % 8 != 0 || !dtype_ok(dtype) || !aligned16(x) || !aligned16(y))
        return fail(ctx, PCV_ERR_INVALID, "pcv_channel_concat: bad argument (C, offset and pitches must be multiples of 8, y must hold the slice)");
    const long total = rows * (C / 8);
    const unsigned grid = (unsigned)((total + 255) / 256);
    hipStream_t st = (hipStream_t)stream;
    if (dtype == PCV_BF16) channel_concat_kernel<PCV_BF16><<<grid, 256, 0, st>>>(x, y, rows, C, x_cpitch, y_cpitch, y_offset);
    else if (dtype == PCV_F16) channel_concat_kernel<PCV_F16><<<grid, 256, 0, st>>>(x, y, rows, C, x_cpitch, y_cpitch, y_offset);
    else channel_concat_kernel<PCV_F32><<<grid, 256, 0, st>>>(x, y, rows, C, x_cpitch, y_cpitch, y_offset);
    HIP_TRY(ctx, hipGetLastError());
    return PCV_OK;
}

int pcv_interpolate(pcv_ctx* ctx, const void* x, void* y, int N, int H, int W, int C, int Ho, int Wo, int bilinear,
                    int align_corners, int dtype, void* stream) {
    if (!ctx) return PCV_ERR_INVALID;
    DeviceGuard device_guard(ctx->device);
    if (!x || !y || N <= 0 || H <= 0 || W <= 0 || C <= 0 || C % 8 != 0 || Ho <= 0 || Wo <= 0 || !dtype_ok(dtype))
        return fail(ctx, PCV_ERR_INVALID, "pcv_interpolate: bad argument (C must be a multiple of 8)");
    const long total = (long)N * Ho * Wo * (C / 8);
    const unsigned grid = (unsigned)((total + 255) / 256);
    hipStream_t st = (hipStream_t)stream;
    if (dtype == PCV_BF16) interpolate_kernel<PCV_BF16><<<grid, 256, 0, st>>>(x, y, N, H, W, C, Ho, Wo, bilinear, align_corners);
    else if (dtype == PCV_F16) interpolate_kernel<PCV_F16><<<grid, 256, 0, st>>>(x, y, N, H, W, C, Ho, Wo, bilinear, align_corners);
    else interpolate_kernel<PCV_F32><<<grid, 256, 0, st>>>(x, y, N, H, W, C, Ho, Wo, bilinear, align_corners);
    HIP_TRY(ctx, hipGetLastError());
    return PCV_OK;
}

int pcv_channel_interleave2(pcv_ctx* ctx, const void* a, const void* b, void* y, long rows, int Ch, int a_cpitch, int b_cpitch,
                            int y_cpitch, int dtype, void* stream) {
    if (!ctx) return PCV_ERR_INVALID;
    DeviceGuard device_guard(ctx->device);
    if (!a || !b || !y || rows <= 0 || Ch <= 0 || a_cpitch < Ch || b_cpitch < Ch || y_cpitch < 2 * Ch || y_cpitch % 8 != 0 ||
        !dtype_ok(dtype))
        return fail(ctx, PCV_ERR_INVALID, "pcv_channel_interleave2: bad argument (y_cpitch must be a multiple of 8 and hold 2*Ch channels)");
    const long total = rows * (y_cpitch / 8);
    const unsigned grid = (unsigned)((total + 255) / 256);
    hipStream_t st = (hipStream_t)stream;
    if (dtype == PCV_BF16) channel_interleave2_kernel<PCV_BF16><<<grid, 256, 0, st>>>(a, b, y, rows, Ch, a_cpitch, b_cpitch, y_cpitch);
    else if (dtype == PCV_F16) channel_interleave2_kernel<PCV_F16><<<grid, 256, 0, st>>>(a, b, y, rows, Ch, a_cpitch, b_cpitch, y_cpitch);
    else channel_interleave2_kernel<PCV_F32><<<grid, 256, 0, st>>>(a, b, y, rows, Ch, a_cpitch, b_cpitch, y_cpitch);
    HIP_TRY(ctx, hipGetLastError());
    return PCV_OK;
}

int pcv_preprocess_u8(pcv_ctx* ctx, const unsigned char* x, void* y, int N, int Hs, int Ws, int C, int top, int left, int H,
                      int W, int wpitch, const float* mean, const float* inv_std, int dtype, void* stream) {
    if (!ctx) return PCV_ERR_INVALID;
    DeviceGuard device_guard(ctx->device);
    if (!x || !y || !mean || !inv_std || N <= 0 || Hs <= 0 || Ws <= 0 || C <= 0 || C > 4 || H <= 0 || W <= 0 || top < 0 ||
        left < 0 || top + H > Hs || left + W > Ws || wpitch < W || !dtype_ok(dtype))
        return fail(ctx, PCV_ERR_INVALID, "pcv_preprocess_u8: bad argument (C <= 4, crop inside the frame, wpitch >= W)");
    const long total = (long)N * H * wpitch;
    const unsigned grid = (unsigned)((total + 255) / 256);
    hipStream_t st = (hipStream_t)stream;
    if (dtype == PCV_BF16) preprocess_u8_kernel<PCV_BF16><<<grid, 256, 0, st>>>(x, y, N, Hs, Ws, C, top, left, H, W, 4, wpitch, mean, inv_std, ctx->ovf);
    else if (dtype == PCV_F16) preprocess_u8_kernel<PCV_F16><<<grid, 256, 0, st>>>(x, y, N, Hs, Ws, C, top, left, H, W, 4, wpitch, mean, inv_std, ctx->ovf);
    else preprocess_u8_kernel<PCV_F32><<<grid, 256, 0, st>>>(x, y, N, Hs, Ws, C, top, left, H, W, 4, wpitch, mean, inv_std, ctx->ovf);
    HIP_TRY(ctx, hipGetLastError());
    return PCV_OK;
}

int pcv_mbconv_supported(const pcv_conv_desc* d_exp, const pcv_conv_desc* d_dw, const pcv_conv_desc* d_proj) {
    return (d_dw && d_proj && mbconv_unsupported(d_exp, *d_dw, *d_proj) == nullptr) ? 1 : 0;
}

int pcv_mbconv_fused(pcv_ctx* ctx, const pcv_conv_desc* d_exp, const pcv_conv_desc* d_dw, const pcv_conv_desc* d_proj,
                     const void* x, const void* packed_exp, const float* scale_e, const float* shift_e, const void* packed_dw,
                     const float* scale_d, const float* shift_d, const void* packed_proj, const float* scale_p,
                     const float* shift_p, const void* residual, void* y, void* stream) {
    if (!ctx) return PCV_ERR_INVALID;
    DeviceGuard device_guard(ctx->device);
    if (!d_dw || !d_proj || !x || !packed_dw || !scale_d || !shift_d || !packed_proj || !scale_p || !shift_p || !y ||
        (d_exp && (!packed_exp || !scale_e || !shift_e)))
        return fail(ctx, PCV_ERR_INVALID, "pcv_mbconv_fused: NULL argument");
    if (const char* why = mbconv_unsupported(d_exp, *d_dw, *d_proj)) return fail(ctx, PCV_ERR_INVALID, std::string("pcv_mbconv_fused: ") + why);
    if (d_proj->has_residual && !residual) return fail(ctx, PCV_ERR_INVALID, "pcv_mbconv_fused: has_residual but residual is NULL");
    if (!aligned16(x) || !aligned16(packed_dw) || !aligned16(packed_proj) || !aligned16(y) || (d_exp && !aligned16(packed_exp)) ||
        (residual && !aligned16(residual)) || !aligned16(scale_d) || !aligned16(shift_d) || !aligned16(scale_p) || !aligned16(shift_p) ||
        (d_exp && (!aligned16(scale_e) || !aligned16(shift_e))))
        return fail(ctx, PCV_ERR_INVALID, "pcv_mbconv_fused: pointers must be 16-byte aligned");
    ConvPlan Pe, Pp;
    const char* why = d_exp ? plan_conv(*d_exp, Pe, false) : nullptr;
    if (!why) why = plan_conv(*d_proj, Pp, false);
    if (why) return fail(ctx, PCV_ERR_INVALID, std::string("pcv_mbconv_fused: ") + why);
    if (Pp.ngb != 1 || (d_exp && Pe.ngb != 1)) return fail(ctx, PCV_ERR_INVALID, "pcv_mbconv_fused: unexpected packed layout");
    MbParams p;
    std::memset(&p, 0, sizeof(p));
    const int S = d_dw->stride_h;
    p.x = x; p.res = d_proj->has_residual ? residual : nullptr; p.y = y; p.ovf = ctx->ovf;
    p.dbg = reinterpret_cast<uint32_t*>(ctx->dbg_ptr);
    p.w_exp = d_exp ? static_cast<const char*>(packed_exp) + Pe.ktab_bytes : nullptr;
    p.w_dw = packed_dw;
    p.w_dwsp = static_cast<const char*>(packed_dw) + dw_taps_bytes(*d_dw);
    p.w_proj = static_cast<const char*>(packed_proj) + Pp.ktab_bytes;
    p.scale_e = scale_e; p.shift_e = shift_e; p.scale_d = scale_d; p.shift_d = shift_d; p.scale_p = scale_p; p.shift_p = shift_p;
    p.N = d_dw->N; p.H = d_dw->H; p.W = d_dw->W; p.Cmid = d_dw->Cin; p.Cin = d_exp ? d_exp->Cin : p.Cmid; p.Cout = d_proj->Cout;
    p.Ho = (p.H - 1) / S + 1; p.Wo = (p.W - 1) / S + 1;
    p.x_bytes = (uint32_t)((long)p.N * p.H * p.W * p.Cin * 2);
    p.y_bytes = (uint32_t)((long)p.N * p.Ho * p.Wo * p.Cout * 2);
    p.wexp_bytes = d_exp ? (uint32_t)Pe.w_bytes : 0;
    p.wdw_bytes = (uint32_t)(9 * p.Cmid * 2);
    p.wproj_bytes = (uint32_t)Pp.w_bytes;
    p.Kpad1 = d_exp ? Pe.Kpad : 0; p.Kpad2 = Pp.Kpad;
    p.ka = d_exp ? (p.Cin + 31) / 32 : 0;
    p.nChunks = (p.Cmid + 31) / 32;
    p.nRowT = Pp.wrows / 16;
    const int TH = S == 1 ? 8 : 4;
    p.tilesH = (p.Ho + TH - 1) / TH; p.tilesW = (p.Wo + 15) / 16;
    p.nTiles = p.N * p.tilesH * p.tilesW;
    p.act_e = d_exp ? d_exp->act : 0; p.act_d = d_dw->act; p.act_p = d_proj->act; p.post = d_proj->post_act;
    if (p.nRowT > 6 || (d_exp && p.Kpad1 < 32 * p.ka) || p.Kpad2 < 32 * p.nChunks)
        return fail(ctx, PCV_ERR_INVALID, "pcv_mbconv_fused: unexpected packed layout");
    int kaw = 0, nrt = 0, rbw = 0;
    const bool wave_shape = d_exp && mbw_shape(p.Cin, p.Cout, S, p.H, p.W, &kaw, &nrt, &rbw);
    const bool block_shape = p.Cout <= 32 && p.Wo >= 24;
    if (wave_shape && ctx->use_mbr) {
        const MbrEntry* e = pick_mbr(d_dw->dtype, nrt, p.act_e == p.act_d ? p.act_e : -1, S, kaw, p.nChunks);
        if (e) {
            const int oc = mbr_out_cols(S, e->nrt);
            p.tilesH = (p.Ho + e->ro - 1) / e->ro; p.tilesW = (p.Wo + oc - 1) / oc;
            const long nT = (long)p.N * p.tilesH * p.tilesW;
            if (nT >= 0x7FFFFFFFl) return fail(ctx, PCV_ERR_TOO_LARGE, "pcv_mbconv_fused: too many tiles; split the batch");
            p.nTiles = (int)nT;
            const unsigned gridr = (unsigned)std::min<long>((nT + e->waves - 1) / e->waves, (long)block_slots(ctx, 1));
            hipLaunchKernelGGL(e->fn, dim3(gridr), dim3(64 * e->waves), mbr_entry_lds(*e, p.nChunks), (hipStream_t)stream, p);
            HIP_TRY(ctx, hipGetLastError());
            return PCV_OK;
        }
    }
    if (wave_shape && (ctx->use_mbw || !block_shape)) {
        const int nblk = rbw > 0 ? rbw : (S == 1 ? 4 : 2);
        auto tiles_of = [&](int tw) { return (long)((p.Ho + nblk * (16 / tw) - 1) / (nblk * (16 / tw))) * ((p.Wo + tw - 1) / tw); };
        int tw = mbw_npt(S, 8, rbw) * tiles_of(8) < mbw_npt(S, 16, rbw) * tiles_of(16) ? 8 : 16;
        if (ctx->use_mbw == 8 || ctx->use_mbw == 16) tw = ctx->use_mbw;
        if (rbw > 0) tw = 16;
        const int nw = mbw_waves(S, nrt, p.nChunks, tw, kaw, rbw);
        if (nw > 0) {
            const int RO = nblk * (16 / tw);
            p.tilesH = (p.Ho + RO - 1) / RO; p.tilesW = (p.Wo + tw - 1) / tw;
            const long nT = (long)p.N * p.tilesH * p.tilesW;
            if (nT >= 0x7FFFFFFFl) return fail(ctx, PCV_ERR_TOO_LARGE, "pcv_mbconv_fused: too many tiles; split the batch");
// ... 43 lines not shown
```

pytorchcv_amd/engine.py:

```python

__all__ = ['NHWC', 'DTYPES', 'default_dtype', 'set_compute_dtype', 'compute_dtype_of', 'Fp16Guard', 'fp16_overflow_count', 'from_nchw', 'to_nchw', 'ConvRunner',
           'BnActRunner', 'maxpool2d', 'avgpool2d', 'avgpool2d_pad', 'global_avgpool', 'se_forward', 'splat_forward', 'channel_slice', 'cat_shuffle2', 'act_code',
           'boundary', 'round8', 'channel_concat_into', 'interpolate', 'add']

import os
import ctypes
import torch
import torch.nn as nn
import torch.nn.functional as F
from . import _lib
from ._lib import ConvDesc

DTYPES = {"fp32": (0, torch.float32), "bf16": (1, torch.bfloat16), "fp16": (2, torch.float16)}
_CODE_OF_TORCH = {torch.float32: 0, torch.bfloat16: 1, torch.float16: 2}
_NAME_OF_TORCH = {torch.float32: "fp32", torch.bfloat16: "bf16", torch.float16: "fp16"}


def default_dtype() -> str:
    d = os.environ.get("PCV_AMD_DTYPE", "auto")
    if d not in DTYPES and d != "auto":
        raise ValueError("PCV_AMD_DTYPE must be one of {}".format(sorted(DTYPES) + ["auto"]))
    return d


# ... 2 lines not shown
        raise ValueError("dtype must be one of {}".format(sorted(DTYPES) + ["auto"]))
    for m in net.modules():
        m._pcv_dtype = dtype
    return net


def stamp_family_dtype(net: nn.Module) -> nn.Module:
    mode = getattr(net, "pcv_16bit", None)
    if mode is not None:
        for m in net.modules():
            if m is not net:
                m.pcv_16bit = mode
    return net


def compute_dtype_of(module: nn.Module) -> str:
    d = getattr(module, "_pcv_dtype", None) or default_dtype()
    if d == "auto":
        d = getattr(module, "pcv_16bit", None) or "bf16"
    return d


class Fp16Guard(object):
    __slots__ = ("slot", "device")

    def __init__(self, device, torch_dtype):
        self.slot = None
        self.device = device
        if torch_dtype == torch.float16:
            self.slot = torch.empty(1, dtype=torch.int32, device=device)
            ctx = _ctx(device)
            _lib.check(_lib.lib().pcv_fp16_guard_begin(ctx, _ptr(self.slot), _stream(device)), ctx)

    def finish(self, y: torch.Tensor) -> torch.Tensor:
        if self.slot is not None:
            if y.dtype != torch.float32 or not y.is_contiguous():
                raise RuntimeError("the fp16 guard poisons a contiguous fp32 result")
            ctx = _ctx(self.device)
            _lib.check(_lib.lib().pcv_fp16_guard_end(ctx, _ptr(self.slot), _ptr(y), y.numel(), _stream(self.device)), ctx)
        return y


def fp16_overflow_count(device) -> int:
    ctx = _ctx(device)
    n = ctypes.c_uint(0)
    _lib.check(_lib.lib().pcv_fp16_overflow_count(ctx, ctypes.byref(n), _stream(device)), ctx)
    return int(n.value)


def round8(c: int) -> int:
    return (int(c) + 7) // 8 * 8


class NHWC(object):
    __slots__ = ("t", "N", "H", "W", "C", "wpitch", "cpitch")

    def __init__(self, t, N, H, W, C, wpitch=None, cpitch=None):
        self.t, self.N, self.H, self.W, self.C = t, N, H, W, C
        self.wpitch = W if wpitch is None else wpitch
        self.cpitch = C if cpitch is None else cpitch

    @property
    def dtype(self):
        return self.t.dtype

    @property
    def device(self):
        return self.t.device

    @property
    def dense(self) -> bool:
        return self.wpitch == self.W and self.cpitch == round8(self.C)

    def size(self, dim=None):
        s = (self.N, self.C, self.H, self.W)
        return s if dim is None else s[dim]


class _ShapeOnly(object):
    __slots__ = ("N", "H", "W", "C", "dtype", "wpitch", "cpitch")

    def __init__(self, N, H, W, C, dtype):
        self.N, self.H, self.W, self.C, self.dtype, self.wpitch, self.cpitch = N, H, W, C, dtype, W, round8(C)


def _stream(device) -> ctypes.c_void_p:
    return ctypes.c_void_p(torch.cuda.current_stream(device).cuda_stream)


def _ctx(device):
    if device.type != "cuda":
        raise RuntimeError("pytorchcv_amd runs on MI355X (gfx950) only: got a tensor on '{}'. Move the model and the input "
                           "to a CUDA/HIP device; there is no CPU path in this package.".format(device))
    idx = device.index if device.index is not None else torch.cuda.current_device()
    return _lib.ctx_for(idx)


def _ptr(t):
    return ctypes.c_void_p(t.data_ptr()) if t is not None else None


class LazyNCHW(NHWC):
    __slots__ = ("src", "_conv", "_dtype_name")

    def __init__(self, x: torch.Tensor, dtype: str):
        N, C, H, W = x.shape
        self.src, self._conv, self._dtype_name = x, None, dtype
        self.N, self.H, self.W, self.C = N, H, W, C
        self.wpitch, self.cpitch = (W + 1) // 2 * 2, 4

    @property
    def t(self):
        if self._conv is None:
            self._conv = from_nchw(self.src, self._dtype_name, stem=True).t
        return self._conv

    @property
    def materialized(self) -> bool:
        return self._conv is not None

    @property
    def dtype(self):
        return DTYPES[self._dtype_name][1]

    @property
    def device(self):
        return self.src.device


def network_input(x: torch.Tensor, dtype: str) -> NHWC:
    if x.dim() != 4:
        raise ValueError("expected a 4-D NCHW tensor")
    if x.shape[1] <= 3 and x.shape[3] % 4 == 0 and STEM_FROM_NCHW:
        return LazyNCHW(x.contiguous().float(), dtype)
    return from_nchw(x, dtype, stem=True)


def from_nchw(x: torch.Tensor, dtype: str, stem: bool = True) -> NHWC:
    if x.dim() != 4:
        raise ValueError("expected a 4-D NCHW tensor")
    x = x.contiguous().float()
    N, C, H, W = x.shape
    code, tdt = DTYPES[dtype]
    if C <= 4 and stem:
        cp, wp = 4, (W + 1) // 2 * 2
    else:
        cp, wp = (C + 7) // 8 * 8, W
    y = torch.empty((N, H, wp, cp), dtype=tdt, device=x.device)
    ctx = _ctx(x.device)
    _lib.check(_lib.lib().pcv_nchw_to_nhwc(ctx, _ptr(x), _ptr(y), N, C, H, W, cp, wp, code, _stream(x.device)), ctx)
    return NHWC(y, N, H, W, C, wpitch=wp, cpitch=cp)


def to_nchw(a: NHWC) -> torch.Tensor:
    if a.wpitch != a.W:
        raise RuntimeError("cannot convert a row-padded input handle back to NCHW")
    y = torch.empty((a.N, a.C, a.H, a.W), dtype=torch.float32, device=a.device)
    ctx = _ctx(a.device)
    _lib.check(_lib.lib().pcv_nhwc_to_nchw(ctx, _ptr(a.t), _ptr(y), a.N, a.C, a.H, a.W, a.cpitch, _CODE_OF_TORCH[a.dtype],
                                           _stream(a.device)), ctx)
    return y


def boundary(module: nn.Module, x, fn, stem: bool = False):
    if isinstance(x, NHWC):
        return fn(x)
# ... 392 lines not shown
    if not x.dense:
        raise RuntimeError("max-pool on a padded handle")
    Ho, Wo = _pool_out(x.H, k, s, p, ceil_mode), _pool_out(x.W, k, s, p, ceil_mode)
    y = torch.empty((x.N, Ho, Wo, x.cpitch), dtype=x.dtype, device=x.device)
    ctx = _ctx(x.device)
    _lib.check(_lib.lib().pcv_maxpool2d(ctx, _ptr(x.t), _ptr(y), x.N, x.H, x.W, x.cpitch, k, s, p, 1 if ceil_mode else 0,
                                        _CODE_OF_TORCH[x.dtype], _stream(x.device)), ctx)
    return NHWC(y, x.N, Ho, Wo, x.C, cpitch=x.cpitch)


def avgpool2d(x: NHWC, k: int, s: int, out_fp32: bool = False) -> NHWC:
    if not x.dense:
        raise RuntimeError("avg-pool on a padded handle")
    if k > x.H or k > x.W:
        raise RuntimeError("AvgPool2d kernel {} larger than the {}x{} map".format(k, x.H, x.W))
    Ho, Wo = (x.H - k) // s + 1, (x.W - k) // s + 1
    y = torch.empty((x.N, Ho, Wo, x.cpitch), dtype=torch.float32 if out_fp32 else x.dtype, device=x.device)
    ctx = _ctx(x.device)
    code = _CODE_OF_TORCH[x.dtype]
    _lib.check(_lib.lib().pcv_avgpool2d(ctx, _ptr(x.t), _ptr(y), x.N, x.H, x.W, x.cpitch, k, s, code, 0 if out_fp32 else code,
                                        _stream(x.device)), ctx)
    return NHWC(y, x.N, Ho, Wo, x.C, cpitch=x.cpitch)


def avgpool2d_pad(x: NHWC, k: int, s: int, p: int = 0, ceil_mode: bool = False, count_include_pad: bool = True) -> NHWC:
    if not x.dense:
        raise RuntimeError("avg-pool on a padded handle")
    Ho, Wo = _pool_out(x.H, k, s, p, ceil_mode), _pool_out(x.W, k, s, p, ceil_mode)
    if Ho <= 0 or Wo <= 0:
        raise RuntimeError("AvgPool2d({}, {}, {}) output of a {}x{} map would be empty".format(k, s, p, x.H, x.W))
    y = torch.empty((x.N, Ho, Wo, x.cpitch), dtype=x.dtype, device=x.device)
    ctx = _ctx(x.device)
    code = _CODE_OF_TORCH[x.dtype]
    _lib.check(_lib.lib().pcv_avgpool2d_pad(ctx, _ptr(x.t), _ptr(y), x.N, x.H, x.W, x.cpitch, k, s, p, 1 if ceil_mode else 0,
                                            1 if count_include_pad else 0, code, code, _stream(x.device)), ctx)
    return NHWC(y, x.N, Ho, Wo, x.C, cpitch=x.cpitch)


FP32_HEAD = os.environ.get("PCV_AMD_FP32_HEAD", "1") != "0"
STEM_FROM_NCHW = os.environ.get("PCV_AMD_STEM_NCHW", "1") != "0"


FUSE_UNITS = os.environ.get("PCV_AMD_FUSE_UNITS", "1") != "0"


def mbconv_fused(exp, exp_act: int, dw, dw_act: int, proj, proj_act: int, x: NHWC, residual, post_act: int):
    if not FUSE_UNITS or not x.dense or not dw.depthwise or proj.depthwise or (exp is not None and exp.depthwise):
        return None
    if any(r is not None and r.pad4 is not None for r in (exp, dw, proj)):
        return None
    for r in (exp, dw, proj):
        if r is not None and r.bn is not None and r.bn.training:
            raise RuntimeError("pytorchcv_amd is an inference path: call net.eval() first (BatchNorm is folded)")
    L, ctx, st = _lib.lib(), _ctx(x.device), _stream(x.device)
    cur = x
    d_exp = None
    if exp is not None:
        d_exp = exp.desc(x, exp_act, 0, False)
        cur = _ShapeOnly(x.N, x.H, x.W, exp.conv.out_channels, x.dtype)
    d_dw = dw.desc(cur, dw_act, 0, False)
    Ho = (cur.H + d_dw.pad_t + d_dw.pad_b - d_dw.dil_h * (d_dw.kh - 1) - 1) // d_dw.stride_h + 1
    Wo = (cur.W + d_dw.pad_l + d_dw.pad_r - d_dw.dil_w * (d_dw.kw - 1) - 1) // d_dw.stride_w + 1
    mid = _ShapeOnly(x.N, Ho, Wo, dw.conv.out_channels, x.dtype)
    d_proj = proj.desc(mid, proj_act, post_act, residual is not None)
    if not L.pcv_mbconv_supported(ctypes.byref(d_exp) if d_exp is not None else None, ctypes.byref(d_dw), ctypes.byref(d_proj)):
        return None
    Cout = d_proj.Cout
    if residual is not None and (not residual.dense or residual.dtype != x.dtype or
                                 tuple(residual.t.shape) != (x.N, Ho, Wo, Cout)):
        raise RuntimeError("residual shape/dtype mismatch")
    if exp is not None:
        exp.prepare(x, d_exp)
    dw.prepare(_PrepHandle(cur, x.device), d_dw)
    proj.prepare(_PrepHandle(mid, x.device), d_proj)
    y = torch.empty((x.N, Ho, Wo, Cout), dtype=x.dtype, device=x.device)
    _lib.check(L.pcv_mbconv_fused(ctx, ctypes.byref(d_exp) if d_exp is not None else None, ctypes.byref(d_dw), ctypes.byref(d_proj),
                                  _ptr(x.t), _ptr(exp.packed) if exp is not None else None,
                                  _ptr(exp.scale) if exp is not None else None, _ptr(exp.shift) if exp is not None else None,
                                  _ptr(dw.packed), _ptr(dw.scale), _ptr(dw.shift), _ptr(proj.packed), _ptr(proj.scale),
                                  _ptr(proj.shift), _ptr(residual.t) if residual is not None else None, _ptr(y), st), ctx)
    return NHWC(y, x.N, Ho, Wo, proj.conv.out_channels, cpitch=Cout)


class _PrepHandle(object):
    __slots__ = ("dtype", "cpitch", "device")

    def __init__(self, shape_only, device):
        self.dtype, self.cpitch, self.device = shape_only.dtype, shape_only.cpitch, device


class BnActRunner(object):
    def __init__(self, bn):
        self.bn = bn
        self._key = None
        self._foreign = False
        self.scale = self.shift = None

    def _state_key(self):
        ts = (self.bn.weight, self.bn.bias, self.bn.running_mean, self.bn.running_var)
        return tuple((t.data_ptr(), t._version) if t is not None else None for t in ts)

    def prepare(self, x: NHWC):
        key = self._state_key()
        if key == self._key:
            return
        if self._foreign:
            raise RuntimeError("this BatchNorm's folded constants were received by parallel.broadcast_packed_state and its local "
                               "parameters changed: call parallel.broadcast_module_state(net) first")
        bn, dev = self.bn, x.device
        if not isinstance(bn, nn.BatchNorm2d):
            raise NotImplementedError("only BatchNorm2d folds to scale/shift, got {}".format(type(bn).__name__))
        if bn.running_mean.device != dev:
            raise RuntimeError("model parameters are on {} but the input is on {}".format(bn.running_mean.device, dev))
        Cl = bn.num_features
        C = round8(Cl)

        def padded(t, fill):
            t = t.detach().float()
            return (F.pad(t, (0, C - Cl), value=fill) if C != Cl else t).contiguous()
        L, ctx, st = _lib.lib(), _ctx(dev), _stream(dev)
        g = padded(bn.weight if bn.weight is not None else torch.ones(Cl, device=dev), 0.0)
        b = padded(bn.bias if bn.bias is not None else torch.zeros(Cl, device=dev), 0.0)
        m = padded(bn.running_mean, 0.0)
        v = padded(bn.running_var, 1.0)
        scale = torch.empty(C, dtype=torch.float32, device=dev)
        shift = torch.empty(C, dtype=torch.float32, device=dev)
        _lib.check(L.pcv_bn_fold(ctx, C, _ptr(g), _ptr(b), _ptr(m), _ptr(v), ctypes.c_float(bn.eps), None, _ptr(scale),
                                 _ptr(shift), st), ctx)
        torch.cuda.current_stream(dev).synchronize()
        self.scale, self.shift, self._key = scale, shift, key

    def adopt_foreign_state(self):
        self._foreign = True

    def local_state_restored(self):
        self._foreign = False
        self._key = None

    def run(self, x: NHWC, act: int) -> NHWC:
        if self.bn.training:
            raise RuntimeError("pytorchcv_amd is an inference path: call net.eval() first (BatchNorm is folded)")
        if x.wpitch != x.W:
            raise RuntimeError("BatchNorm + activation on a row-padded handle")
        if x.C != self.bn.num_features:
            raise RuntimeError("BatchNorm2d expects {} channels, got {}".format(self.bn.num_features, x.C))
        self.prepare(x)
        CP = round8(x.C)
        y = torch.empty((x.N, x.H, x.W, CP), dtype=x.dtype, device=x.device)
        ctx = _ctx(x.device)
        _lib.check(_lib.lib().pcv_bn_act(ctx, _ptr(x.t), _ptr(self.scale), _ptr(self.shift), _ptr(y), x.N * x.H * x.W, CP,
                                         x.cpitch, act, _CODE_OF_TORCH[x.dtype], _stream(x.device)), ctx)
        return NHWC(y, x.N, x.H, x.W, x.C, cpitch=CP)


def global_avgpool(x: NHWC, out_fp32: bool = False) -> NHWC:
    if not x.dense:
        raise RuntimeError("avg-pool on a padded handle")
    y = torch.empty((x.N, 1, 1, x.cpitch), dtype=torch.float32 if out_fp32 else x.dtype, device=x.device)
    ctx = _ctx(x.device)
    code = _CODE_OF_TORCH[x.dtype]
    _lib.check(_lib.lib().pcv_global_avgpool(ctx, _ptr(x.t), _ptr(y), x.N, x.H * x.W, x.cpitch, code, 0 if out_fp32 else code,
                                             _stream(x.device)), ctx)
    return NHWC(y, x.N, 1, 1, x.C, cpitch=x.cpitch)


def se_forward(x: NHWC, w1, b1, w2, b2, mid_act: int, out_act: int, residual: NHWC | None, post_act: int) -> NHWC:
# ... 47 lines not shown
```

pytorchcv_amd/models/common/conv.py:

```python

__all__ = ['conv1x1', 'conv3x3', 'depthwise_conv3x3', 'ConvBlock', 'conv1x1_block', 'conv3x3_block', 'conv5x5_block',
           'conv7x7_block', 'dwconv_block', 'dwconv3x3_block', 'dwconv5x5_block', 'DwsConvBlock', 'dwsconv3x3_block', 'BareConv', 'PreConvBlock',
           'pre_conv1x1_block', 'pre_conv3x3_block', 'conv_block_pair', 'conv_block_maxpool', 'mbconv_chain']

import torch.nn as nn
from .activ import lambda_relu, create_activation_layer
from .norm import lambda_batchnorm2d, create_normalization_layer
from ... import engine


class BareConv(nn.Conv2d):
    def forward(self, x, out_fp32: bool = False, act: int = 0):
        if getattr(self, "_pcv_runner", None) is None:
            self._pcv_runner = engine.ConvRunner(self, None)
        return engine.boundary(self, x, lambda a: self._pcv_runner.run(a, act=act, out_fp32=out_fp32))


def conv1x1(in_channels, out_channels, stride=1, groups=1, bias=False):
    return BareConv(in_channels=in_channels, out_channels=out_channels, kernel_size=1, stride=stride, groups=groups, bias=bias)


def conv3x3(in_channels, out_channels, stride=1, padding=1, dilation=1, groups=1, bias=False):
    return BareConv(in_channels=in_channels, out_channels=out_channels, kernel_size=3, stride=stride, padding=padding,
                    dilation=dilation, groups=groups, bias=bias)


def depthwise_conv3x3(channels, stride=1, padding=1, dilation=1, bias=False):
    return BareConv(in_channels=channels, out_channels=channels, kernel_size=3, stride=stride, padding=padding,
                    dilation=dilation, groups=channels, bias=bias)


class ConvBlock(nn.Module):
    def __init__(self, in_channels, out_channels, kernel_size, stride=1, padding=0, dilation=1, groups=1, bias=False,
                 normalization=lambda_batchnorm2d(), activation=lambda_relu()):
        super(ConvBlock, self).__init__()
        self.normalize = (normalization is not None)
        self.activate = (activation is not None)
        self.use_pad = (isinstance(padding, (list, tuple)) and (len(padding) == 4))
        self._pad4 = tuple(int(p) for p in padding) if self.use_pad else None
        self.conv = nn.Conv2d(in_channels=in_channels, out_channels=out_channels, kernel_size=kernel_size, stride=stride,
                              padding=(0 if self.use_pad else padding), dilation=dilation, groups=groups, bias=bias)
        if self.normalize:
            self.bn = create_normalization_layer(normalization=normalization, num_features=out_channels)
            if self.bn is None:
                self.normalize = False
            else:
                assert isinstance(self.bn, nn.Module)
        if self.activate:
            self.activ = create_activation_layer(activation)
            if self.activ is None:
                self.activate = False
            else:
                assert isinstance(self.activ, nn.Module)
        self._pcv_runner = None

    def forward(self, x, residual=None, post_act=None, pad4=None, out=None):
        if self._pcv_runner is None:
            self._pcv_runner = engine.ConvRunner(self.conv, self.bn if self.normalize else None, pad4=self._pad4)
        act = engine.act_code(self.activ) if self.activate else 0
        pact = engine.act_code(post_act)
        return engine.boundary(self, x, lambda a: self._pcv_runner.run(a, act=act, residual=residual, post_act=pact,
                                                                       pad4=pad4, out=out))


def conv_block_maxpool(block, x, pool):
    if isinstance(block, ConvBlock) and isinstance(x, engine.NHWC) and not block.use_pad:
        if block._pcv_runner is None:
            block._pcv_runner = engine.ConvRunner(block.conv, block.bn if block.normalize else None, pad4=block._pad4)
        y = block._pcv_runner.run_maxpool(x, engine.act_code(block.activ) if block.activate else 0, pool.kernel_size,
                                          pool.stride, pool.padding, pool.ceil_mode)
        if y is not None:
            return y
    return pool(block(x))


def conv_block_pair(first, x, residual, post_act, second, id_block=None, x0=None):
    if not (isinstance(first, ConvBlock) and isinstance(second, ConvBlock) and isinstance(x, engine.NHWC)):
        return None
    for blk in (first, second) + ((id_block,) if id_block is not None else ()):
        if not isinstance(blk, ConvBlock):
            return None
        if blk._pcv_runner is None:
            blk._pcv_runner = engine.ConvRunner(blk.conv, blk.bn if blk.normalize else None, pad4=blk._pad4)
    if id_block is not None:
        if id_block.activate or not isinstance(x0, engine.NHWC):
            return None
        return first._pcv_runner.run_pair_idconv(x, x0, id_block._pcv_runner, engine.act_code(first.activ) if first.activate else 0,
                                                 engine.act_code(post_act), second._pcv_runner,
                                                 engine.act_code(second.activ) if second.activate else 0)
    return first._pcv_runner.run_pair(x, residual, engine.act_code(first.activ) if first.activate else 0,
                                      engine.act_code(post_act), second._pcv_runner,
                                      engine.act_code(second.activ) if second.activate else 0)


def mbconv_chain(exp_block, dw_block, proj_block, x, residual=None, post_act=None):
    blocks = [b for b in (exp_block, dw_block, proj_block) if b is not None]
    if not isinstance(x, engine.NHWC) or not all(isinstance(b, ConvBlock) for b in blocks):
        return None
    for blk in blocks:
        if blk._pcv_runner is None:
            blk._pcv_runner = engine.ConvRunner(blk.conv, blk.bn if blk.normalize else None, pad4=blk._pad4)

    def code(blk):
        return engine.act_code(blk.activ) if blk.activate else 0
    return engine.mbconv_fused(exp_block._pcv_runner if exp_block is not None else None,
                               code(exp_block) if exp_block is not None else 0, dw_block._pcv_runner, code(dw_block),
                               proj_block._pcv_runner, code(proj_block), x, residual, engine.act_code(post_act))


def conv1x1_block(padding=0, **kwargs):
    return ConvBlock(kernel_size=1, padding=padding, **kwargs)


def conv3x3_block(padding=1, **kwargs):
    return ConvBlock(kernel_size=3, padding=padding, **kwargs)


def conv5x5_block(padding=2, **kwargs):
    return ConvBlock(kernel_size=5, padding=padding, **kwargs)


def conv7x7_block(padding=3, **kwargs):
    return ConvBlock(kernel_size=7, padding=padding, **kwargs)


def dwconv_block(out_channels, padding=1, **kwargs):
    return ConvBlock(out_channels=out_channels, padding=padding, groups=out_channels, **kwargs)


def dwconv3x3_block(padding=1, **kwargs):
    return dwconv_block(kernel_size=3, padding=padding, **kwargs)


def dwconv5x5_block(padding=2, **kwargs):
    return dwconv_block(kernel_size=5, padding=padding, **kwargs)


class DwsConvBlock(nn.Module):
    def __init__(self, in_channels, out_channels, kernel_size, stride=1, padding=0, dilation=1, bias=False,
                 dw_normalization=lambda_batchnorm2d(), pw_normalization=lambda_batchnorm2d(), dw_activation=lambda_relu(),
                 pw_activation=lambda_relu()):
        super(DwsConvBlock, self).__init__()
        self.dw_conv = dwconv_block(in_channels=in_channels, out_channels=in_channels, kernel_size=kernel_size, stride=stride,
                                    padding=padding, dilation=dilation, bias=bias, normalization=dw_normalization,
                                    activation=dw_activation)
        self.pw_conv = conv1x1_block(in_channels=in_channels, out_channels=out_channels, bias=bias,
                                     normalization=pw_normalization, activation=pw_activation)

    def _run(self, a):
        y = mbconv_chain(None, self.dw_conv, self.pw_conv, a)
        return y if y is not None else self.pw_conv(self.dw_conv(a))

    def forward(self, x):
        return engine.boundary(self, x, self._run)


def dwsconv3x3_block(padding=1, **kwargs):
    return DwsConvBlock(kernel_size=3, padding=padding, **kwargs)


class PreConvBlock(nn.Module):
    def __init__(self, in_channels, out_channels, kernel_size, stride, padding, dilation=1, bias=False,
                 normalization=lambda_batchnorm2d(), activation=lambda_relu(), return_preact=False):
        super(PreConvBlock, self).__init__()
        self.normalize = (normalization is not None)
        self.activate = (activation is not None)
        self.return_preact = return_preact
        if self.normalize:
            self.bn = create_normalization_layer(normalization=normalization, num_features=in_channels)
            if self.bn is None:
                self.normalize = False
            else:
                assert isinstance(self.bn, nn.BatchNorm2d)
        if self.activate:
            self.activ = create_activation_layer(activation)
            if self.activ is None:
                self.activate = False
# ... 51 lines not shown
```

pytorchcv_amd/models/resnet.py:

```python

__all__ = ['ResNet', 'resnet10', 'resnet12', 'resnet14', 'resnetbc14b', 'resnet16', 'resnet18', 'resnet26', 'resnetbc26b',
           'resnet34', 'resnetbc38b', 'resnet50', 'resnet50b', 'resnet101', 'resnet101b', 'resnet152', 'resnet152b',
           'ResBlock', 'ResBottleneck', 'ResUnit', 'ResStage', 'ResInitBlock', 'get_resnet']

import torch.nn as nn
from .common.activ import lambda_relu
from .common.norm import lambda_batchnorm2d
from .common.conv import conv1x1_block, conv3x3_block, conv7x7_block, conv_block_pair, conv_block_maxpool
from ._tail import MaxPool2dNHWC, AvgPool2dNHWC, LinearHead, run_net, maybe_load_pretrained, init_conv_params, DEFAULT_ROOT
from .. import engine


class ResBlock(nn.Module):
    def __init__(self, in_channels, out_channels, stride, bias=False, normalization=lambda_batchnorm2d(),
                 activation=lambda_relu(), final_activation=None):
        super(ResBlock, self).__init__()
        self.conv1 = conv3x3_block(in_channels=in_channels, out_channels=out_channels, stride=stride, bias=bias,
                                   normalization=normalization, activation=activation)
        self.conv2 = conv3x3_block(in_channels=out_channels, out_channels=out_channels, bias=bias,
                                   normalization=normalization, activation=final_activation)

    def forward(self, x, residual=None, post_act=None):
        return engine.boundary(self, x, lambda a: self.conv2(self.conv1(a), residual=residual, post_act=post_act))


class ResBottleneck(nn.Module):
    def __init__(self, in_channels, out_channels, stride, padding=1, dilation=1, bias=False,
                 normalization=lambda_batchnorm2d(), conv1_stride=False, bottleneck_factor=4, activation=lambda_relu(),
                 final_activation=None):
        super(ResBottleneck, self).__init__()
        mid_channels = out_channels // bottleneck_factor
        self.conv1 = conv1x1_block(in_channels=in_channels, out_channels=mid_channels, stride=(stride if conv1_stride else 1),
                                   bias=bias, normalization=normalization, activation=activation)
        self.conv2 = conv3x3_block(in_channels=mid_channels, out_channels=mid_channels,
                                   stride=(1 if conv1_stride else stride), padding=padding, dilation=dilation, bias=bias,
                                   normalization=normalization, activation=activation)
        self.conv3 = conv1x1_block(in_channels=mid_channels, out_channels=out_channels, bias=bias,
                                   normalization=normalization, activation=final_activation)

    def forward(self, x, residual=None, post_act=None):
        return engine.boundary(self, x, lambda a: self.conv3(self.conv2(self.conv1(a)), residual=residual, post_act=post_act))


class ResUnit(nn.Module):
    def __init__(self, in_channels, out_channels, stride=1, padding=1, dilation=1, bias=False,
                 normalization=lambda_batchnorm2d(), bottleneck=True, conv1_stride=False, activation=lambda_relu(),
                 final_body_activation=None, final_activation=lambda_relu()):
        super(ResUnit, self).__init__()
        self.resize_identity = (in_channels != out_channels) or (stride != 1)
        if bottleneck:
            self.body = ResBottleneck(in_channels=in_channels, out_channels=out_channels, stride=stride, padding=padding,
                                      dilation=dilation, bias=bias, normalization=normalization, conv1_stride=conv1_stride,
                                      activation=activation, final_activation=final_body_activation)
        else:
            self.body = ResBlock(in_channels=in_channels, out_channels=out_channels, stride=stride, bias=bias,
                                 normalization=normalization, activation=activation, final_activation=final_body_activation)
        if self.resize_identity:
            self.identity_conv = conv1x1_block(in_channels=in_channels, out_channels=out_channels, stride=stride, bias=bias,
                                               normalization=normalization, activation=None)
        self.activ = final_activation()

    def _run(self, a):
        identity = self.identity_conv(a) if self.resize_identity else a
        return self.body(a, residual=identity, post_act=self.activ)

    def run_chained(self, a, conv1_out=None, next_unit=None):
        body = self.body
        y = body.conv2(conv1_out if conv1_out is not None else body.conv1(a))
        if next_unit is not None and self.resize_identity:
            pair = conv_block_pair(body.conv3, y, None, self.activ, next_unit.body.conv1, id_block=self.identity_conv, x0=a)
            if pair is not None:
                return pair
        identity = self.identity_conv(a) if self.resize_identity else a
        if next_unit is not None:
            pair = conv_block_pair(body.conv3, y, identity, self.activ, next_unit.body.conv1)
            if pair is not None:
                return pair
        return body.conv3(y, residual=identity, post_act=self.activ), None

    def forward(self, x):
        return engine.boundary(self, x, self._run)


class ResStage(nn.Sequential):
    def forward(self, x):
        units = list(self.children())
        chainable = all((isinstance(u, ResUnit) and isinstance(u.body, ResBottleneck)) or getattr(u, "pcv_chainable", False) for u in units)
        if not isinstance(x, engine.NHWC) or not chainable:
            return super(ResStage, self).forward(x)
        conv1_out = None
        for i, unit in enumerate(units):
            x, conv1_out = unit.run_chained(x, conv1_out, units[i + 1] if i + 1 < len(units) else None)
        return x


class ResInitBlock(nn.Module):
    def __init__(self, in_channels, out_channels, normalization=lambda_batchnorm2d()):
        super(ResInitBlock, self).__init__()
        self.conv = conv7x7_block(in_channels=in_channels, out_channels=out_channels, stride=2, normalization=normalization)
        self.pool = MaxPool2dNHWC(kernel_size=3, stride=2, padding=1)

    def forward(self, x):
        return engine.boundary(self, x, lambda a: conv_block_maxpool(self.conv, a, self.pool), stem=True)


class ResNet(nn.Module):
    def __init__(self, channels, init_block_channels, bottleneck, conv1_stride, in_channels=3, in_size=(224, 224),
                 num_classes=1000):
        super(ResNet, self).__init__()
        self.in_size = in_size
        self.num_classes = num_classes
        self.features = nn.Sequential()
        self.features.add_module("init_block", ResInitBlock(in_channels=in_channels, out_channels=init_block_channels))
        in_channels = init_block_channels
        for i, channels_per_stage in enumerate(channels):
            stage = ResStage()
            for j, out_channels in enumerate(channels_per_stage):
                stride = 2 if (j == 0) and (i != 0) else 1
                stage.add_module("unit{}".format(j + 1), ResUnit(in_channels=in_channels, out_channels=out_channels,
                                                                 stride=stride, bottleneck=bottleneck,
                                                                 conv1_stride=conv1_stride))
                in_channels = out_channels
            self.features.add_module("stage{}".format(i + 1), stage)
        self.features.add_module("final_pool", AvgPool2dNHWC(kernel_size=7, stride=1, fp32_out=True))
        self.output = LinearHead(in_features=in_channels, out_features=num_classes)
        init_conv_params(self)

    def forward(self, x):
        return run_net(self, x, self.output)


_LAYERS = {10: [1, 1, 1, 1], 12: [2, 1, 1, 1], 16: [2, 2, 2, 1], 18: [2, 2, 2, 2], 34: [3, 4, 6, 3], 50: [3, 4, 6, 3],
           101: [3, 4, 23, 3], 152: [3, 8, 36, 3], 200: [3, 24, 36, 3]}


def resnet_layers(blocks, bottleneck, what="ResNet"):
    if blocks == 14:
        layers = [1, 1, 1, 1] if bottleneck else [2, 2, 1, 1]
    elif blocks == 26:
        layers = [2, 2, 2, 2] if bottleneck else [3, 3, 3, 3]
    elif blocks == 38 and bottleneck:
        layers = [3, 3, 3, 3]
    elif blocks in _LAYERS:
        layers = _LAYERS[blocks]
    else:
        raise ValueError("Unsupported {} with number of blocks: {}".format(what, blocks))
    assert (sum(layers) * (3 if bottleneck else 2) + 2 == blocks)
    return layers


def get_resnet(blocks, bottleneck=None, conv1_stride=True, width_scale=1.0, model_name=None, pretrained=False,
# ... 81 lines not shown
```

Baseline: 89810 images/sec.

## Fuse whole ResNet bottleneck unit into one kernel for 1024-channel stage

Adds a single kernel that runs the 1x1 reduce, the 3x3, and the 1x1 expand convolutions of an identity bottleneck unit per image. Intermediate activations stay in LDS, so they are never written to or read back from HBM. The resnet unit scheduler uses this path when it is supported, and gives up the conv3+next-conv1 pair fusion when the next unit can fuse whole. The cost is one workgroup per image, which limits parallelism to the batch size, plus heavy LDS and register pressure.

```diff
diff --git a/include/pcv_amd.h b/include/pcv_amd.h
--- a/include/pcv_amd.h
+++ b/include/pcv_amd.h
@@ -136,6 +136,11 @@
                                   const void* x, const void* packed1, const float* scale1, const float* shift1, void* y1,
                                   const void* packed2, const float* scale2, const float* shift2, void* y2, void* stream);
 
+int pcv_bottleneck_supported(const pcv_conv_desc* d1, const pcv_conv_desc* d2, const pcv_conv_desc* d3);
+int pcv_bottleneck_fused(pcv_ctx* ctx, const pcv_conv_desc* d1, const pcv_conv_desc* d2, const pcv_conv_desc* d3, const void* x,
+                         const void* packed1, const float* scale1, const float* shift1, const void* packed2, const float* scale2,
+                         const float* shift2, const void* packed3, const float* scale3, const float* shift3, void* y, void* stream);
+
 int pcv_mbconv_supported(const pcv_conv_desc* d_exp, const pcv_conv_desc* d_dw, const pcv_conv_desc* d_proj);
 int pcv_mbconv_fused(pcv_ctx* ctx, const pcv_conv_desc* d_exp, const pcv_conv_desc* d_dw, const pcv_conv_desc* d_proj,
                      const void* x, const void* packed_exp, const float* scale_e, const float* shift_e,
diff --git a/pytorchcv_amd/_lib.py b/pytorchcv_amd/_lib.py
--- a/pytorchcv_amd/_lib.py
+++ b/pytorchcv_amd/_lib.py
@@ -82,6 +82,9 @@
     "pcv_conv1x1_pair_idconv_supported": (_I, [ctypes.POINTER(ConvDesc), ctypes.POINTER(ConvDesc), ctypes.POINTER(ConvDesc)]),
     "pcv_conv1x1_pair_idconv_fused": (_I, [_VP, ctypes.POINTER(ConvDesc), ctypes.POINTER(ConvDesc), ctypes.POINTER(ConvDesc),
                                            _VP, _VP, _VP, _VP, _VP, _VP, _VP, _VP, _VP, _VP, _VP, _VP, _VP, _VP]),
+    "pcv_bottleneck_supported": (_I, [ctypes.POINTER(ConvDesc), ctypes.POINTER(ConvDesc), ctypes.POINTER(ConvDesc)]),
+    "pcv_bottleneck_fused": (_I, [_VP, ctypes.POINTER(ConvDesc), ctypes.POINTER(ConvDesc), ctypes.POINTER(ConvDesc), _VP, _VP, _VP, _VP,
+                                  _VP, _VP, _VP, _VP, _VP, _VP, _VP, _VP]),
     "pcv_mbconv_supported": (_I, [ctypes.POINTER(ConvDesc), ctypes.POINTER(ConvDesc), ctypes.POINTER(ConvDesc)]),
     "pcv_mbconv_fused": (_I, [_VP, ctypes.POINTER(ConvDesc), ctypes.POINTER(ConvDesc), ctypes.POINTER(ConvDesc), _VP, _VP, _VP, _VP,
                               _VP, _VP, _VP, _VP, _VP, _VP, _VP, _VP, _VP]),
diff --git a/pytorchcv_amd/csrc/bneck_16bit.hip b/pytorchcv_amd/csrc/bneck_16bit.hip
--- /dev/null
+++ b/pytorchcv_amd/csrc/bneck_16bit.hip
@@ -0,0 +1,3 @@
+#include "bneck_conv.hpp"
+template __global__ void bneck_kernel<PCV_BF16>(const BneckParams);
+template __global__ void bneck_kernel<PCV_F16>(const BneckParams);
diff --git a/pytorchcv_amd/csrc/bneck_conv.hpp b/pytorchcv_amd/csrc/bneck_conv.hpp
--- /dev/null
+++ b/pytorchcv_amd/csrc/bneck_conv.hpp
@@ -0,0 +1,466 @@
+#pragma once
+#include <type_traits>
+#include <utility>
+#include "pcv_common.hpp"
+#include "igemm_conv.hpp"
+#include "d3q_conv.hpp"
+#include "d3i_conv.hpp"
+#include "d1i_conv.hpp"
+
+struct BneckParams {
+    const void* x;
+    void* y;
+    const void* w1;
+    const void* w2;
+    const void* w3;
+    const float* scale1;
+    const float* shift1;
+    const float* scale2;
+    const float* shift2;
+    const float* scale3;
+    const float* shift3;
+    uint32_t w1_bytes, w2_bytes, w3_bytes;
+    int N, H, W, HW;
+    float inv_w;
+    uint32_t* ovf;
+    uint32_t* dbg;
+};
+
+struct BneckCfg {
+    typedef D1ICfgT<1024> A;
+    typedef D3ICfgT<256> B;
+    static constexpr int THREADS = 256;
+    static constexpr int C1 = 1024, CM = 256;
+    static constexpr int NB = 13;
+    static constexpr int KH3 = CM / 32;
+    static constexpr int PASSES = C1 / 256;
+    static constexpr int KT3 = KH3 * PASSES;
+    static constexpr int W3BYTES = KH3 * 4096;
+    static constexpr int LDS = A::LDS > B::LDS ? A::LDS : B::LDS;
+    static_assert(A::NBLK == NB && B::NBLK == NB && A::PITCH == B::PITCH, "one pixel-block count, one slot pitch");
+    static_assert(KT3 % 4 == 0, "weight ring slots are compile-time");
+    static_assert(LDS <= 160 * 1024, "LDS");
+};
+
+#if defined(__HIP_DEVICE_COMPILE__)
+template <int DT>
+__device__ __forceinline__ void bneck_body(const BneckParams& p, char* smem) {
+    typedef BneckCfg G;
+    typedef typename G::A GA;
+    typedef typename G::B GB;
+    typedef typename Mma<DT>::frag frag;
+    typedef const __attribute__((address_space(3))) frag* lds_fptr;
+    typedef __attribute__((address_space(3))) u32x4* lds_wptr;
+    constexpr int NB = G::NB;
+    const int tid = threadIdx.x, lane = tid & 63;
+    const int wave = __builtin_amdgcn_readfirstlane(tid >> 6);
+    const int fr = lane & 15, fq = lane >> 4;
+    const uint32_t lds0 = (uint32_t)__builtin_amdgcn_readfirstlane((int)(uint32_t)(size_t)PCV_LDS(smem));
+    const int n = (int)blockIdx.x;
+    const int W = p.W, HW = p.HW;
+#ifdef BNECK_CYCLES
+    uint64_t cyc__[5];
+    cyc__[0] = __builtin_amdgcn_s_memtime();
+#endif
+
+    const uint32_t imgBytes = (uint32_t)(HW * G::C1 * 2);
+    const __amdgpu_buffer_rsrc_t xrsrc = __builtin_amdgcn_make_buffer_rsrc(const_cast<char*>(reinterpret_cast<const char*>(p.x)) + (size_t)n * imgBytes, 0,
+                                                                           imgBytes, 0x00020000);
+    const __amdgpu_buffer_rsrc_t yrsrc = __builtin_amdgcn_make_buffer_rsrc(reinterpret_cast<char*>(p.y) + (size_t)n * imgBytes, 0, imgBytes, 0x00020000);
+    const uint32_t wlane = (uint32_t)(lane * 16);
+    const int chw = wave * 64 + 8 * fq;
+
+    constexpr uint32_t kDump = (uint32_t)(GB::NSLOT * GB::PITCH);
+    static_assert(GB::NSLOT * GB::PITCH + GB::PITCH <= GB::LDS, "the dump slot lies inside the allocation");
+    auto slot_of = [&](int mb) __attribute__((always_inline)) -> uint32_t {
+        int f = fr;
+        asm volatile("" : "+v"(f));
+        const int pix = 16 * mb + f;
+        const int py = (int)(((float)pix + 0.5f) * p.inv_w);
+        const uint32_t s = (uint32_t)((py * (GB::GW - W) + pix + GB::GW + 1) * GB::PITCH);
+        return pix < HW ? s : kDump;
+    };
+    auto lds_out = [&](int mb, int g, const u32x4& o) __attribute__((always_inline)) {
+        *reinterpret_cast<lds_wptr>((size_t)(lds0 + slot_of(mb) + (uint32_t)((chw + 32 * g) * 2))) = o;
+    };
+
+    {
+        typedef GA Q;
+        const __amdgpu_buffer_rsrc_t wrsrc = __builtin_amdgcn_make_buffer_rsrc(const_cast<void*>(p.w1), 0, p.w1_bytes, 0x00020000);
+        const uint32_t wbase = (uint32_t)(wave * Q::WBYTES);
+        frag Wf[Q::WRING][4];
+        auto wload = [&](int kh, auto SLc) __attribute__((always_inline)) {
+            constexpr int sl = decltype(SLc)::value;
+#pragma unroll
+            for (int nb = 0; nb < 4; ++nb) {
+                const u32x4 v = __builtin_amdgcn_raw_buffer_load_b128(wrsrc, wlane + (uint32_t)(nb * 1024), wbase + (uint32_t)(kh * 4096), 0);
+                Wf[sl][nb] = __builtin_bit_cast(frag, v);
+            }
+        };
+        d3i_unroll([&](auto KHc) __attribute__((always_inline)) { wload(decltype(KHc)::value, KHc); }, std::make_integer_sequence<int, Q::PFW>{});
+
+        const int spix = tid >> 3, sc8 = tid & 7;
+        const uint32_t sbase = (uint32_t)((spix * Q::CIN + sc8 * 8) * 2);
+        const uint32_t srow = (uint32_t)(32 * Q::CIN * 2);
+        const uint32_t slds = lds0 + (uint32_t)(spix * Q::PITCH + sc8 * 16);
+        auto sload = [&](int s, u32x4 (&buf)[Q::SPT]) __attribute__((always_inline)) {
+#pragma unroll
+            for (int i = 0; i < Q::SPT; ++i) buf[i] = __builtin_amdgcn_raw_buffer_load_b128(xrsrc, sbase + (uint32_t)i * srow + (uint32_t)(s * 128), 0, 0);
+        };
+        auto swrite = [&](int s, const u32x4 (&buf)[Q::SPT]) __attribute__((always_inline)) {
+#pragma unroll
+            for (int i = 0; i < Q::SPT; ++i) *reinterpret_cast<lds_wptr>((size_t)(slds + (uint32_t)(32 * i * Q::PITCH + (s % Q::NS) * 128))) = buf[i];
+        };
+        u32x4 sb[2][Q::SPT];
+        {
+            u32x4 pb[2][Q::SPT];
+            sload(0, pb[0]);
+            sload(1, pb[1]);
+            sload(2, sb[0]);
+            sload(3, sb[1]);
+            swrite(0, pb[0]);
+            swrite(1, pb[1]);
+        }
+        uint32_t ab[NB];
+#pragma unroll
+        for (int mb = 0; mb < NB; ++mb) ab[mb] = lds0 + (uint32_t)((16 * mb + fr) * Q::PITCH + fq * 16);
+
+        f32x4 acc[NB][4];
+#pragma unroll
+        for (int mb = 0; mb < NB; ++mb)
+#pragma unroll
+            for (int nb = 0; nb < 4; ++nb) acc[mb][nb] = (f32x4){0.f, 0.f, 0.f, 0.f};
+
+        asm volatile("s_waitcnt lgkmcnt(0)" ::: "memory");
+        d3q_sync();
+
+        frag Pf[2][NB];
+        auto pread = [&](auto KHc, auto MBc) __attribute__((always_inline)) {
+            constexpr int kh = decltype(KHc)::value, mb = decltype(MBc)::value;
+            Pf[kh & 1][mb] = *reinterpret_cast<lds_fptr>((size_t)ab[mb] + (size_t)(((kh >> 1) % Q::NS) * 128 + (kh & 1) * 64));
+        };
+        auto preads = [&](auto KHc) __attribute__((always_inline)) {
+            d3i_unroll([&](auto MBc) __attribute__((always_inline)) { pread(KHc, MBc); }, std::make_integer_sequence<int, NB>{});
+        };
+        preads(std::integral_constant<int, 0>{});
+        f32x4 es[2][2], eh[2][2];
+        auto step = [&](auto KHc) __attribute__((always_inline)) {
+            constexpr int kh = decltype(KHc)::value, s = kh >> 1;
+            constexpr bool first = (kh & 1) == 0;
+            constexpr bool wr = first && s + 2 < Q::SLICES;
+            constexpr bool ld = first && s + 4 < Q::SLICES;
+            if constexpr (wr) swrite(s + 2, sb[s & 1]);
+            if constexpr (kh + 1 < Q::KH) preads(std::integral_constant<int, kh + 1>{});
+            if constexpr (kh + Q::PFW < Q::KH) {
+                wload(kh + Q::PFW, std::integral_constant<int, (kh + Q::PFW) % Q::WRING>{});
+            } else if constexpr (kh + Q::PFW == Q::KH) {
+#pragma unroll
+                for (int g = 0; g < 2; ++g) {
+                    es[g][0] = *reinterpret_cast<const f32x4*>(p.scale1 + chw + 32 * g); es[g][1] = *reinterpret_cast<const f32x4*>(p.scale1 + chw + 32 * g + 4);
+                    eh[g][0] = *reinterpret_cast<const f32x4*>(p.shift1 + chw + 32 * g); eh[g][1] = *reinterpret_cast<const f32x4*>(p.shift1 + chw + 32 * g + 4);
+                }
+            }
+            if constexpr (ld) sload(s + 4, sb[s & 1]);
+#pragma unroll
+            for (int mb = 0; mb < NB; ++mb)
+#pragma unroll
+                for (int nb = 0; nb < 4; ++nb) acc[mb][nb] = Mma<DT>::run(Wf[kh % Q::WRING][nb], Pf[kh & 1][mb], acc[mb][nb]);
+            d3i_unroll([&](auto MBc) __attribute__((always_inline)) {
+                constexpr int mb = decltype(MBc)::value;
+                __builtin_amdgcn_sched_group_barrier(0x008, 4, 0);
+                if constexpr (!wr) {
+                    __builtin_amdgcn_sched_group_barrier(0x100, 1, 0);
+                } else if constexpr (mb < Q::SPT) {
+                    __builtin_amdgcn_sched_group_barrier(0x200, 1, 0);
+                } else {
+                    constexpr int RG = NB - Q::SPT;
+                    __builtin_amdgcn_sched_group_barrier(0x100, (NB * (mb - Q::SPT + 1)) / RG - (NB * (mb - Q::SPT)) / RG, 0);
+                }
+                if constexpr ((mb + 1) * 4 / NB != mb * 4 / NB) __builtin_amdgcn_sched_group_barrier(0x020, 1, 0);
+                if constexpr (ld && mb >= NB - Q::SPT) __builtin_amdgcn_sched_group_barrier(0x020, 1, 0);
+            }, std::make_integer_sequence<int, NB>{});
+            __builtin_amdgcn_sched_barrier(0);
+            if constexpr (first && s + 1 < Q::SLICES && s >= 1) {
+                asm volatile("s_waitcnt lgkmcnt(%0)" ::"n"(NB) : "memory");
+                d3q_sync();
+            }
+        };
+        d3i_unroll([&](auto KHc) __attribute__((always_inline)) { step(KHc); }, std::make_integer_sequence<int, Q::KH>{});
+
+        asm volatile("s_waitcnt lgkmcnt(0)" ::: "memory");
+        d3q_sync();
+        {
+            const int gy = tid >> 4, gx = tid & 15;
+            if (!((unsigned)(gy - 1) < (unsigned)p.H && (unsigned)(gx - 1) < (unsigned)W)) {
+                const u32x4 z = {0u, 0u, 0u, 0u};
+#pragma unroll
+                for (int i = 0; i < 32; ++i) *reinterpret_cast<lds_wptr>((size_t)(lds0 + (uint32_t)(tid * GB::PITCH + i * 16))) = z;
+            }
+        }
+        F16Guard<DT> guard;
+#pragma unroll
+        for (int g = 0; g < 2; ++g) {
+            const f32x4 es0 = es[g][0], es1 = es[g][1], eh0 = eh[g][0], eh1 = eh[g][1];
+#pragma unroll
+            for (int mb = 0; mb < NB; ++mb) {
+                u32x4 o;
+#pragma unroll
+                for (int e = 0; e < 4; ++e) {
+                    const int hf = e >> 1, k0 = 2 * (e & 1);
+                    const f32x4& a = acc[mb][2 * g + hf];
+                    const f32x4& sc = hf == 0 ? es0 : es1;
+                    const f32x4& sh = hf == 0 ? eh0 : eh1;
+                    float v0 = a[k0] * sc[k0] + sh[k0], v1 = a[k0 + 1] * sc[k0 + 1] + sh[k0 + 1];
+                    v0 = __builtin_elementwise_maximum(v0, 0.f);
+                    v1 = __builtin_elementwise_maximum(v1, 0.f);
+                    guard.see2(v0, v1);
+                    o[e] = pack2<DT>(v0, v1);
+                }
+                lds_out(mb, g, o);
+            }
+        }
+        guard.commit(p.ovf);
+        asm volatile("s_waitcnt lgkmcnt(0)" ::: "memory");
+        d3q_sync();
+    }
+#ifdef BNECK_CYCLES
+    cyc__[1] = __builtin_amdgcn_s_memtime();
+#endif
+
+    {
+        typedef GB Q;
+        const __amdgpu_buffer_rsrc_t wrsrc = __builtin_amdgcn_make_buffer_rsrc(const_cast<void*>(p.w2), 0, p.w2_bytes, 0x00020000);
+        const uint32_t wbase = (uint32_t)(wave * Q::WBYTES);
+        frag Wf[Q::WRING][4];
+        auto wload = [&](int kh, auto SLc) __attribute__((always_inline)) {
+            constexpr int sl = decltype(SLc)::value;
+#pragma unroll
+            for (int nb = 0; nb < 4; ++nb) {
+                const u32x4 v = __builtin_amdgcn_raw_buffer_load_b128(wrsrc, wlane + (uint32_t)(nb * 1024), wbase + (uint32_t)(kh * 4096), 0);
+                Wf[sl][nb] = __builtin_bit_cast(frag, v);
+            }
+        };
+        wload(0, std::integral_constant<int, 0>{});
+        wload(1, std::integral_constant<int, 1>{});
+        wload(2, std::integral_constant<int, 2>{});
+        static_assert(Q::PFW == 3, "the three loads above");
+
+        uint32_t ab[NB];
+#pragma unroll
+        for (int mb = 0; mb < NB; ++mb)
+            ab[mb] = lds0 + (16 * mb + fr < HW ? slot_of(mb) - (uint32_t)(Q::ROWB + Q::PITCH) : 0u) + (uint32_t)(fq * 16);
+
+        f32x4 acc[NB][4];
+#pragma unroll
+        for (int mb = 0; mb < NB; ++mb)
+#pragma unroll
+            for (int nb = 0; nb < 4; ++nb) acc[mb][nb] = (f32x4){0.f, 0.f, 0.f, 0.f};
+
+        frag Pf[2][NB];
+        auto pread = [&](auto Jc, auto MBc) __attribute__((always_inline)) {
+            constexpr int j = decltype(Jc)::value, mb = decltype(MBc)::value;
+            Pf[j & 1][mb] = *reinterpret_cast<lds_fptr>((size_t)ab[mb] + (size_t)Q::pimm(j));
+        };
+        auto preads = [&](auto Jc) __attribute__((always_inline)) {
+            d3i_unroll([&](auto MBc) __attribute__((always_inline)) { pread(Jc, MBc); }, std::make_integer_sequence<int, NB>{});
+        };
+        preads(std::integral_constant<int, 0>{});
+        f32x4 es[2][2], eh[2][2];
+        auto step = [&](auto Rc, auto Jc) __attribute__((always_inline)) {
+            constexpr int r = decltype(Rc)::value, j = decltype(Jc)::value, kh = r * Q::JR + j;
+            if constexpr (kh + 1 < Q::KH) preads(std::integral_constant<int, j + 1>{});
+            if constexpr (kh + Q::PFW < Q::KH) {
+                wload(kh + Q::PFW, std::integral_constant<int, (j + Q::PFW) % Q::WRING>{});
+            } else if constexpr (kh + Q::PFW == Q::KH) {
+#pragma unroll
+                for (int g = 0; g < 2; ++g) {
+                    es[g][0] = *reinterpret_cast<const f32x4*>(p.scale2 + chw + 32 * g); es[g][1] = *reinterpret_cast<const f32x4*>(p.scale2 + chw + 32 * g + 4);
+                    eh[g][0] = *reinterpret_cast<const f32x4*>(p.shift2 + chw + 32 * g); eh[g][1] = *reinterpret_cast<const f32x4*>(p.shift2 + chw + 32 * g + 4);
+                }
+            }
+#pragma unroll
+            for (int mb = 0; mb < NB; ++mb)
+#pragma unroll
+                for (int nb = 0; nb < 4; ++nb) acc[mb][nb] = Mma<DT>::run(Wf[j % Q::WRING][nb], Pf[j & 1][mb], acc[mb][nb]);
+            d3i_unroll([&](auto MBc) __attribute__((always_inline)) {
+                constexpr int mb = decltype(MBc)::value;
+                __builtin_amdgcn_sched_group_barrier(0x008, 4, 0);
+                __builtin_amdgcn_sched_group_barrier(0x100, 1, 0);
+                if constexpr ((mb + 1) * 4 / NB != mb * 4 / NB) __builtin_amdgcn_sched_group_barrier(0x020, 1, 0);
+            }, std::make_integer_sequence<int, NB>{});
+            __builtin_amdgcn_sched_barrier(0);
+        };
+        auto row = [&](auto Rc) __attribute__((always_inline)) {
+            d3i_unroll([&](auto Jc) __attribute__((always_inline)) { step(Rc, Jc); }, std::make_integer_sequence<int, Q::JR>{});
+#pragma unroll
+            for (int mb = 0; mb < NB; ++mb) ab[mb] += (uint32_t)Q::ROWB;
+        };
+        row(std::integral_constant<int, 0>{});
+        row(std::integral_constant<int, 1>{});
+        row(std::integral_constant<int, 2>{});
+
+        asm volatile("s_waitcnt lgkmcnt(0)" ::: "memory");
+        d3q_sync();
+        F16Guard<DT> guard;
+#pragma unroll
+        for (int g = 0; g < 2; ++g) {
+            const f32x4 es0 = es[g][0], es1 = es[g][1], eh0 = eh[g][0], eh1 = eh[g][1];
+#pragma unroll
+            for (int mb = 0; mb < NB; ++mb) {
+                u32x4 o;
+#pragma unroll
+                for (int e = 0; e < 4; ++e) {
+                    const int hf = e >> 1, k0 = 2 * (e & 1);
+                    const f32x4& a = acc[mb][2 * g + hf];
+                    const f32x4& sc = hf == 0 ? es0 : es1;
+                    const f32x4& sh = hf == 0 ? eh0 : eh1;
+                    float v0 = a[k0] * sc[k0] + sh[k0], v1 = a[k0 + 1] * sc[k0 + 1] + sh[k0 + 1];
+                    v0 = __builtin_elementwise_maximum(v0, 0.f);
+                    v1 = __builtin_elementwise_maximum(v1, 0.f);
+                    guard.see2(v0, v1);
+                    o[e] = pack2<DT>(v0, v1);
+                }
+                lds_out(mb, g, o);
+            }
+        }
+        guard.commit(p.ovf);
+        asm volatile("s_waitcnt lgkmcnt(0)" ::: "memory");
+        d3q_sync();
+    }
+#ifdef BNECK_CYCLES
+    cyc__[2] = __builtin_amdgcn_s_memtime();
+#endif
+
+    {
+        const __amdgpu_buffer_rsrc_t wrsrc = __builtin_amdgcn_make_buffer_rsrc(const_cast<void*>(p.w3), 0, p.w3_bytes, 0x00020000);
+        constexpr int KT = G::KT3, KH = G::KH3, PFW = 3, WRING = 4;
+        frag Wf[WRING][4];
+        auto wload = [&](int t, auto SLc) __attribute__((always_inline)) {
+            constexpr int sl = decltype(SLc)::value;
+#pragma unroll
+            for (int nb = 0; nb < 4; ++nb) {
+                const u32x4 v = __builtin_amdgcn_raw_buffer_load_b128(wrsrc, wlane + (uint32_t)(nb * 1024),
+                                                                      (uint32_t)(((t / KH) * 4 + wave) * G::W3BYTES + (t % KH) * 4096), 0);
+                Wf[sl][nb] = __builtin_bit_cast(frag, v);
+            }
+        };
+        wload(0, std::integral_constant<int, 0>{});
+        wload(1, std::integral_constant<int, 1>{});
+        wload(2, std::integral_constant<int, 2>{});
+
+        uint32_t ab[NB];
+#pragma unroll
+        for (int mb = 0; mb < NB; ++mb) ab[mb] = lds0 + slot_of(mb) + (uint32_t)(fq * 16);
+
+        f32x4 acc[NB][4];
+#pragma unroll
+        for (int mb = 0; mb < NB; ++mb)
+#pragma unroll
+            for (int nb = 0; nb < 4; ++nb) acc[mb][nb] = (f32x4){0.f, 0.f, 0.f, 0.f};
+
+        frag Pf[2][NB];
+        auto pread = [&](auto Tc, auto MBc) __attribute__((always_inline)) {
+            constexpr int t = decltype(Tc)::value, mb = decltype(MBc)::value, k = t % KH;
+            Pf[t & 1][mb] = *reinterpret_cast<lds_fptr>((size_t)ab[mb] + (size_t)((k >> 1) * 128 + (k & 1) * 64));
+        };
+        auto preads = [&](auto Tc) __attribute__((always_inline)) {
+            d3i_unroll([&](auto MBc) __attribute__((always_inline)) { pread(Tc, MBc); }, std::make_integer_sequence<int, NB>{});
+        };
+        preads(std::integral_constant<int, 0>{});
+        f32x4 es[2][2], eh[2][2];
+        F16Guard<DT> guard;
+        auto epilogue = [&](int pass) __attribute__((always_inline)) {
+            u32x4 rr[2][NB];
+#pragma unroll
+            for (int g = 0; g < 2; ++g)
+#pragma unroll
+                for (int mb = 0; mb < NB; ++mb) {
+                    const int pix = 16 * mb + fr, ch0 = 256 * pass + chw + 32 * g;
+                    const uint32_t roff = pix < HW ? (uint32_t)((pix * G::C1 + ch0) * 2) : 0x80000000u;
+                    rr[g][mb] = __builtin_amdgcn_raw_buffer_load_b128(xrsrc, roff, 0, 0);
+                }
+#pragma unroll
+            for (int g = 0; g < 2; ++g) {
+                const int ch0 = 256 * pass + chw + 32 * g;
+                const f32x4 es0 = es[g][0], es1 = es[g][1], eh0 = eh[g][0], eh1 = eh[g][1];
+#pragma unroll
+                for (int mb = 0; mb < NB; ++mb) {
+                    u32x4 o;
+#pragma unroll
+                    for (int e = 0; e < 4; ++e) {
+                        const int hf = e >> 1, k0 = 2 * (e & 1);
+                        const f32x4& a = acc[mb][2 * g + hf];
+                        const f32x4& sc = hf == 0 ? es0 : es1;
+                        const f32x4& sh = hf == 0 ? eh0 : eh1;
+                        float v0 = a[k0] * sc[k0] + sh[k0], v1 = a[k0 + 1] * sc[k0 + 1] + sh[k0 + 1];
+                        float lo, hi;
+                        unpack2<DT>(rr[g][mb][e], lo, hi);
+                        v0 += lo;
+                        v1 += hi;
+                        v0 = __builtin_elementwise_maximum(v0, 0.f);
+                        v1 = __builtin_elementwise_maximum(v1, 0.f);
+                        guard.see2(v0, v1);
+                        o[e] = pack2<DT>(v0, v1);
+                    }
+                    const int pix = 16 * mb + fr;
+                    const uint32_t boff = pix < HW ? (uint32_t)((pix * G::C1 + ch0) * 2) : 0x80000000u;
+                    __builtin_amdgcn_raw_buffer_store_b128(o, yrsrc, boff, 0, 0);
+                }
+            }
+        };
+        auto step = [&](auto Tc) __attribute__((always_inline)) {
+            constexpr int t = decltype(Tc)::value, k = t % KH, pass = t / KH;
+            if constexpr (t + 1 < KT && k + 1 < KH) preads(std::integral_constant<int, t + 1>{});
+            if constexpr (t + PFW < KT) wload(t + PFW, std::integral_constant<int, (t + PFW) % WRING>{});
+            if constexpr (k == KH - PFW) {
+#pragma unroll
+                for (int g = 0; g < 2; ++g) {
+                    const int ch0 = 256 * pass + chw + 32 * g;
+                    es[g][0] = *reinterpret_cast<const f32x4*>(p.scale3 + ch0); es[g][1] = *reinterpret_cast<const f32x4*>(p.scale3 + ch0 + 4);
+                    eh[g][0] = *reinterpret_cast<const f32x4*>(p.shift3 + ch0); eh[g][1] = *reinterpret_cast<const f32x4*>(p.shift3 + ch0 + 4);
+                }
+            }
+#pragma unroll
+            for (int mb = 0; mb < NB; ++mb)
+#pragma unroll
+                for (int nb = 0; nb < 4; ++nb) acc[mb][nb] = Mma<DT>::run(Wf[t % WRING][nb], Pf[t & 1][mb], acc[mb][nb]);
+            d3i_unroll([&](auto MBc) __attribute__((always_inline)) {
+                constexpr int mb = decltype(MBc)::value;
+                __builtin_amdgcn_sched_group_barrier(0x008, 4, 0);
+                __builtin_amdgcn_sched_group_barrier(0x100, 1, 0);
+                if constexpr ((mb + 1) * 4 / NB != mb * 4 / NB) __builtin_amdgcn_sched_group_barrier(0x020, 1, 0);
+            }, std::make_integer_sequence<int, NB>{});
+            __builtin_amdgcn_sched_barrier(0);
+            if constexpr (k == KH - 1) {
+                epilogue(pass);
+                if constexpr (t + 1 < KT) {
+                    preads(std::integral_constant<int, t + 1>{});
+#pragma unroll
+                    for (int mb = 0; mb < NB; ++mb)
+#pragma unroll
+                        for (int nb = 0; nb < 4; ++nb) acc[mb][nb] = (f32x4){0.f, 0.f, 0.f, 0.f};
+                }
+            }
+        };
+        d3i_unroll([&](auto Tc) __attribute__((always_inline)) { step(Tc); }, std::make_integer_sequence<int, KT>{});
+        guard.commit(p.ovf);
+    }
+#ifdef BNECK_CYCLES
+    __builtin_amdgcn_s_waitcnt(0x0070);
+    cyc__[3] = __builtin_amdgcn_s_memtime();
+    if (p.dbg != nullptr && lane == 0) {
+        uint32_t* d = p.dbg + (blockIdx.x * 4 + wave) * 8;
+        for (int i = 0; i < 3; ++i) d[i] = (uint32_t)(cyc__[i + 1] - cyc__[i]);
+        d[7] = 1u;
+    }
+#endif
+}
+#endif
+
+template <int DT>
+__global__ __launch_bounds__(256, 1) void bneck_kernel(const BneckParams p) {
+#if defined(__HIP_DEVICE_COMPILE__)
+    extern __shared__ __attribute__((aligned(16))) char smem[];
+    bneck_body<DT>(p, smem);
+#endif
+}
diff --git a/pytorchcv_amd/csrc/pcv_api.hip b/pytorchcv_amd/csrc/pcv_api.hip
--- a/pytorchcv_amd/csrc/pcv_api.hip
+++ b/pytorchcv_amd/csrc/pcv_api.hip
@@ -14,6 +14,7 @@
 #include "d3k_conv.hpp"
 #include "d3i_conv.hpp"
 #include "d1i_conv.hpp"
+#include "bneck_conv.hpp"
 #include "p1r_conv.hpp"
 #include "stem_conv.hpp"
 #include "pair1x1.hpp"
@@ -59,6 +60,8 @@
 extern template __global__ void d1i_kernel<PCV_F16, 1024>(const D3Params);
 extern template __global__ void d1i_kernel<PCV_BF16, 2048>(const D3Params);
 extern template __global__ void d1i_kernel<PCV_F16, 2048>(const D3Params);
+extern template __global__ void bneck_kernel<PCV_BF16>(const BneckParams);
+extern template __global__ void bneck_kernel<PCV_F16>(const BneckParams);
 #define P1R_DECLARE(CW, CIN)                                                       \
     extern template __global__ void p1r_kernel<PCV_BF16, CW, CIN>(const D3Params); \
     extern template __global__ void p1r_kernel<PCV_F16, CW, CIN>(const D3Params);
@@ -147,6 +150,7 @@
     bool gconv = false;
     bool d3i = false;
     bool d1i = false;
+    bool bnk3 = false;
     size_t d3i_off = 0;
     size_t gconv_off = 0;
     std::vector<uint32_t> ktab;
@@ -249,7 +253,10 @@
     P.d1i = !P.conv3 && !P.pair && !P.stem && P.ES == 2 && d.kh == 1 && d.kw == 1 && d.groups == 1 && d.stride_h == 1 && d.stride_w == 1 &&
             d.pad_t == 0 && d.pad_l == 0 && d.pad_b == 0 && d.pad_r == 0 && (d.Cin == 1024 || d.Cin == 2048) &&
             d.Cout % 64 == 0 && d.out_dtype == d.dtype && P.wrows >= d.Cout && P.Kpad == d.Cin && P.ngb == 1;
-    if (P.d1i) {
+    P.bnk3 = !P.conv3 && !P.pair && !P.stem && P.ES == 2 && d.kh == 1 && d.kw == 1 && d.groups == 1 && d.stride_h == 1 && d.stride_w == 1 &&
+             d.pad_t == 0 && d.pad_l == 0 && d.pad_b == 0 && d.pad_r == 0 && d.Cin == BneckCfg::CM && d.Cout == BneckCfg::C1 &&
+             d.out_dtype == d.dtype && P.wrows >= d.Cout && P.Kpad == d.Cin && P.ngb == 1;
+    if (P.d1i || P.bnk3) {
         P.d3i_off = (P.total_bytes + 15) / 16 * 16;
         P.total_bytes = P.d3i_off + (size_t)(d.Cout / 64) * (size_t)(d.Cin / 32) * 4096;
     }
@@ -468,6 +475,7 @@
                                  {reinterpret_cast<const void*>(d3i_kernel<PCV_BF16, 512>), reinterpret_cast<const void*>(d3i_kernel<PCV_F16, 512>)}};
 static const void* kD1I[2][2] = {{reinterpret_cast<const void*>(d1i_kernel<PCV_BF16, 1024>), reinterpret_cast<const void*>(d1i_kernel<PCV_F16, 1024>)},
                                  {reinterpret_cast<const void*>(d1i_kernel<PCV_BF16, 2048>), reinterpret_cast<const void*>(d1i_kernel<PCV_F16, 2048>)}};
+static const void* kBneck[2] = {reinterpret_cast<const void*>(bneck_kernel<PCV_BF16>), reinterpret_cast<const void*>(bneck_kernel<PCV_F16>)};
 static const void* kD3K[2] = {reinterpret_cast<const void*>(d3k_kernel<PCV_BF16>), reinterpret_cast<const void*>(d3k_kernel<PCV_F16>)};
 #define P1R_ROW(CW, CIN)                                                                   \
     {P1RCfg<CW, CIN>::BM, P1RCfg<CW, CIN>::BP, P1RCfg<CW, CIN>::LDS,                       \
@@ -482,6 +490,7 @@
         for (int t = 0; t < 2; ++t) HIP_TRY(ctx, hipFuncSetAttribute(kD1I[i][t], hipFuncAttributeMaxDynamicSharedMemorySize, D1ICfgT<1024>::LDS));
     for (int t = 0; t < 2; ++t) HIP_TRY(ctx, hipFuncSetAttribute(kD3I[0][t], hipFuncAttributeMaxDynamicSharedMemorySize, D3ICfgT<256>::LDS));
     for (int t = 0; t < 2; ++t) HIP_TRY(ctx, hipFuncSetAttribute(kD3I[1][t], hipFuncAttributeMaxDynamicSharedMemorySize, D3ICfgT<512>::LDS));
+    for (int t = 0; t < 2; ++t) HIP_TRY(ctx, hipFuncSetAttribute(kBneck[t], hipFuncAttributeMaxDynamicSharedMemorySize, BneckCfg::LDS));
     for (int i = 0; i < kD3WCount; ++i)
         for (int t = 0; t < 2; ++t)
             HIP_TRY(ctx, hipFuncSetAttribute(kD3W[i].fn[t], hipFuncAttributeMaxDynamicSharedMemorySize, kD3W[i].lds));
@@ -548,6 +557,7 @@
 static int pair_lds(int pb, bool idc = false) { return (idc ? 6 : 3) * 16 * pb * 64 * 2 + 16 * 1024 * pb + (idc ? 4096 : 0); }
 static int g_pair_idc_blocks_per_cu = 1;
 static int g_pair_blocks_per_cu[2] = {1, 1};
+static int g_bneck = 0;
 static int g_wpair_mask = 3;
 static int g_wpair_blocks_per_cu[4] = {1, 1, 1, 1};
 struct WPairLaunch { const void* fn; int threads, lds, tileP; bool gate_in_lds; };
@@ -832,6 +842,7 @@
     else if (k == "pair_pb") ctx->pair_pb = value;
     else if (k == "mbw_wide") g_mbw_wide = value;
     else if (k == "wpair") g_wpair_mask = value;
+    else if (k == "bneck") g_bneck = value;
     else if (k == "max_blocks") ctx->max_blocks = value;
     else if (k == "d3x3") ctx->use_d3x3 = value;
     else if (k == "d3w") ctx->use_d3w = value;
@@ -1064,7 +1075,7 @@
         } else if (bf) pack_gconv_kernel<PCV_BF16><<<ggrid, 256, 0, s>>>(w, gout, d->Cin, P.Cg_in);
         else pack_gconv_kernel<PCV_F16><<<ggrid, 256, 0, s>>>(w, gout, d->Cin, P.Cg_in);
     }
-    if (P.d3i || P.d1i) {
+    if (P.d3i || P.d1i || P.bnk3) {
         const int total = (int)((P.total_bytes - P.d3i_off) / 16);
         pack_d3i_kernel<<<(unsigned)((total + 255) / 256), 256, 0, s>>>(reinterpret_cast<const u32x4*>(pp.out),
                                                                         reinterpret_cast<u32x4*>(static_cast<char*>(packed) + P.d3i_off), P.Kpad, total);
@@ -2172,6 +2183,68 @@
     else if (dtype == PCV_F16) preprocess_u8_kernel<PCV_F16><<<grid, 256, 0, st>>>(x, y, N, Hs, Ws, C, top, left, H, W, 4, wpitch, mean, inv_std, ctx->ovf);
     else preprocess_u8_kernel<PCV_F32><<<grid, 256, 0, st>>>(x, y, N, Hs, Ws, C, top, left, H, W, 4, wpitch, mean, inv_std, ctx->ovf);
     HIP_TRY(ctx, hipGetLastError());
+    return PCV_OK;
+}
+
+static const char* bneck_unsupported(const pcv_conv_desc& a, const pcv_conv_desc& b, const pcv_conv_desc& c) {
+    if (desc_stale(a) || desc_stale(b) || desc_stale(c)) return kStaleDesc;
+    if (!g_bneck) return "not switched on (pcv_set_tuning(\"bneck\", 1))";
+    auto dense_io = [](const pcv_conv_desc& d) {
+        return d.groups == 1 && d.dil_h == 1 && d.dil_w == 1 && d.out_dtype == d.dtype && (d.x_cpitch == 0 || d.x_cpitch == d.Cin) &&
+               (d.x_wpitch == 0 || d.x_wpitch == d.W) && (d.y_cpitch == 0 || d.y_cpitch == d.Cout);
+    };
+    auto is1x1 = [](const pcv_conv_desc& d) {
+        return d.kh == 1 && d.kw == 1 && d.stride_h == 1 && d.stride_w == 1 && d.pad_t == 0 && d.pad_l == 0 && d.pad_b == 0 && d.pad_r == 0;
+    };
+    if (!dense_io(a) || !dense_io(b) || !dense_io(c) || !is1x1(a) || !is1x1(c)) return "conv1 and conv3 must be plain 1x1 stride 1";
+    if (b.kh != 3 || b.kw != 3 || b.stride_h != 1 || b.stride_w != 1 || b.pad_t != 1 || b.pad_l != 1 || b.pad_b != 1 || b.pad_r != 1)
+        return "conv2 must be 3x3 / stride 1 / padding 1";
+    if (a.dtype != b.dtype || a.dtype != c.dtype || (a.dtype != PCV_BF16 && a.dtype != PCV_F16)) return "16-bit storage only";
+    if (a.Cin != BneckCfg::C1 || a.Cout != BneckCfg::CM || b.Cin != BneckCfg::CM || b.Cout != BneckCfg::CM || c.Cin != BneckCfg::CM ||
+        c.Cout != BneckCfg::C1)
+        return "only 1024 -> 256 -> 256 -> 1024 is instantiated";
+    if (a.N != b.N || a.N != c.N || a.H != b.H || a.H != c.H || a.W != b.W || a.W != c.W) return "shapes do not chain";
+    if (a.N < 1 || a.H < 1 || a.W < 1 || a.H > BneckCfg::B::MAXW || a.W > BneckCfg::B::MAXW) return "maps up to 14 x 14";
+    if (a.act != PCV_ACT_RELU || a.post_act != PCV_ACT_NONE || a.has_residual || b.act != PCV_ACT_RELU || b.post_act != PCV_ACT_NONE ||
+        b.has_residual || c.act != PCV_ACT_NONE || c.post_act != PCV_ACT_RELU || !c.has_residual)
+        return "the unit must be BN-ReLU, BN-ReLU, BN + identity, ReLU";
+    return nullptr;
+}
+
+int pcv_bottleneck_supported(const pcv_conv_desc* d1, const pcv_conv_desc* d2, const pcv_conv_desc* d3) {
+    return (d1 && d2 && d3 && bneck_unsupported(*d1, *d2, *d3) == nullptr) ? 1 : 0;
+}
+
+int pcv_bottleneck_fused(pcv_ctx* ctx, const pcv_conv_desc* d1, const pcv_conv_desc* d2, const pcv_conv_desc* d3, const void* x,
+                         const void* packed1, const float* scale1, const float* shift1, const void* packed2, const float* scale2,
+                         const float* shift2, const void* packed3, const float* scale3, const float* shift3, void* y, void* stream) {
+    if (!ctx) return PCV_ERR_INVALID;
+    DeviceGuard device_guard(ctx->device);
+    if (!d1 || !d2 || !d3 || !x || !packed1 || !scale1 || !shift1 || !packed2 || !scale2 || !shift2 || !packed3 || !scale3 || !shift3 || !y)
+        return fail(ctx, PCV_ERR_INVALID, "pcv_bottleneck_fused: NULL argument");
+    if (const char* why = bneck_unsupported(*d1, *d2, *d3)) return fail(ctx, PCV_ERR_INVALID, std::string("pcv_bottleneck_fused: ") + why);
+    if (!aligned16(x) || !aligned16(y) || !aligned16(packed1) || !aligned16(packed2) || !aligned16(packed3) || !aligned16(scale1) ||
+        !aligned16(shift1) || !aligned16(scale2) || !aligned16(shift2) || !aligned16(scale3) || !aligned16(shift3))
+        return fail(ctx, PCV_ERR_INVALID, "pcv_bottleneck_fused: pointers must be 16-byte aligned");
+    ConvPlan P1, P2, P3;
+    const char* why = plan_conv(*d1, P1, false);
+    if (!why) why = plan_conv(*d2, P2, false);
+    if (!why) why = plan_conv(*d3, P3, false);
+    if (why) return fail(ctx, PCV_ERR_INVALID, std::string("pcv_bottleneck_fused: ") + why);
+    if (!P1.d1i || !P2.d3i || !P3.bnk3) return fail(ctx, PCV_ERR_INVALID, "pcv_bottleneck_fused: unexpected packed layout");
+    BneckParams q;
+    std::memset(&q, 0, sizeof(q));
+    q.x = x; q.y = y; q.ovf = ctx->ovf;
+    q.w1 = static_cast<const char*>(packed1) + P1.d3i_off; q.w1_bytes = (uint32_t)(P1.total_bytes - P1.d3i_off);
+    q.w2 = static_cast<const char*>(packed2) + P2.d3i_off; q.w2_bytes = (uint32_t)(P2.total_bytes - P2.d3i_off);
+    q.w3 = static_cast<const char*>(packed3) + P3.d3i_off; q.w3_bytes = (uint32_t)(P3.total_bytes - P3.d3i_off);
+    q.scale1 = scale1; q.shift1 = shift1; q.scale2 = scale2; q.shift2 = shift2; q.scale3 = scale3; q.shift3 = shift3;
+    q.N = d1->N; q.H = d1->H; q.W = d1->W; q.HW = d1->H * d1->W;
+    q.inv_w = 1.0f / (float)d1->W;
+    q.dbg = reinterpret_cast<uint32_t*>(ctx->dbg_ptr);
+    void* args[] = {&q};
+    HIP_TRY(ctx, hipLaunchKernel(kBneck[d1->dtype == PCV_BF16 ? 0 : 1], dim3((unsigned)d1->N), dim3(BneckCfg::THREADS), args,
+                                 (size_t)BneckCfg::LDS, (hipStream_t)stream));
     return PCV_OK;
 }
 
diff --git a/pytorchcv_amd/engine.py b/pytorchcv_amd/engine.py
--- a/pytorchcv_amd/engine.py
+++ b/pytorchcv_amd/engine.py
@@ -108,6 +108,9 @@
 
     def __init__(self, N, H, W, C, dtype):
         self.N, self.H, self.W, self.C, self.dtype, self.wpitch, self.cpitch = N, H, W, C, dtype, W, round8(C)
+
+
+ShapeOnly = _ShapeOnly
 
 
 def _stream(device) -> ctypes.c_void_p:
@@ -666,6 +669,32 @@
     return NHWC(y, x.N, Ho, Wo, proj.conv.out_channels, cpitch=Cout)
 
 
+def bottleneck_fused(c1, act1: int, c2, act2: int, c3, act3: int, x: NHWC, post_act: int, check_only: bool = False):
+    if not FUSE_UNITS or not (isinstance(x, NHWC) and x.dense or check_only and isinstance(x, _ShapeOnly)) or any(r.depthwise or r.pad4 is not None for r in (c1, c2, c3)):
+        return None
+    if any(r.bn is not None and r.bn.training for r in (c1, c2, c3)):
+        raise RuntimeError("pytorchcv_amd is an inference path: call net.eval() first (BatchNorm is folded)")
+    L = _lib.lib()
+    d1 = c1.desc(x, act1, 0, False)
+    s1 = _ShapeOnly(x.N, x.H, x.W, c1.conv.out_channels, x.dtype)
+    d2 = c2.desc(s1, act2, 0, False)
+    s2 = _ShapeOnly(x.N, x.H, x.W, c2.conv.out_channels, x.dtype)
+    d3 = c3.desc(s2, act3, post_act, True)
+    if not L.pcv_bottleneck_supported(ctypes.byref(d1), ctypes.byref(d2), ctypes.byref(d3)):
+        return None
+    if check_only:
+        return True
+    c1.prepare(x, d1)
+    c2.prepare(_PrepHandle(s1, x.device), d2)
+    c3.prepare(_PrepHandle(s2, x.device), d3)
+    ctx, st = _ctx(x.device), _stream(x.device)
+    y = torch.empty((x.N, x.H, x.W, d3.Cout), dtype=x.dtype, device=x.device)
+    _lib.check(L.pcv_bottleneck_fused(ctx, ctypes.byref(d1), ctypes.byref(d2), ctypes.byref(d3), _ptr(x.t), _ptr(c1.packed),
+                                      _ptr(c1.scale), _ptr(c1.shift), _ptr(c2.packed), _ptr(c2.scale), _ptr(c2.shift),
+                                      _ptr(c3.packed), _ptr(c3.scale), _ptr(c3.shift), _ptr(y), st), ctx)
+    return NHWC(y, x.N, x.H, x.W, c3.conv.out_channels, cpitch=d3.Cout)
+
+
 class _PrepHandle(object):
     __slots__ = ("dtype", "cpitch", "device")
 
diff --git a/pytorchcv_amd/models/common/conv.py b/pytorchcv_amd/models/common/conv.py
--- a/pytorchcv_amd/models/common/conv.py
+++ b/pytorchcv_amd/models/common/conv.py
@@ -1,7 +1,8 @@
 
 __all__ = ['conv1x1', 'conv3x3', 'depthwise_conv3x3', 'ConvBlock', 'conv1x1_block', 'conv3x3_block', 'conv5x5_block',
            'conv7x7_block', 'dwconv_block', 'dwconv3x3_block', 'dwconv5x5_block', 'DwsConvBlock', 'dwsconv3x3_block', 'BareConv', 'PreConvBlock',
-           'pre_conv1x1_block', 'pre_conv3x3_block', 'conv_block_pair', 'conv_block_maxpool', 'mbconv_chain']
+           'pre_conv1x1_block', 'pre_conv3x3_block', 'conv_block_pair', 'conv_block_maxpool', 'mbconv_chain',
+           'bottleneck_unit']
 
 import torch.nn as nn
 from .activ import lambda_relu, create_activation_layer
@@ -93,6 +94,20 @@
                                       engine.act_code(second.activ) if second.activate else 0)
 
 
+def bottleneck_unit(conv1, conv2, conv3, x, post_act, check_only=False):
+    blocks = (conv1, conv2, conv3)
+    if not isinstance(x, (engine.NHWC, engine.ShapeOnly)) or not all(isinstance(b, ConvBlock) for b in blocks):
+        return None
+    for blk in blocks:
+        if blk._pcv_runner is None:
+            blk._pcv_runner = engine.ConvRunner(blk.conv, blk.bn if blk.normalize else None, pad4=blk._pad4)
+
+    def code(blk):
+        return engine.act_code(blk.activ) if blk.activate else 0
+    return engine.bottleneck_fused(conv1._pcv_runner, code(conv1), conv2._pcv_runner, code(conv2), conv3._pcv_runner, code(conv3), x,
+                                   engine.act_code(post_act), check_only=check_only)
+
+
 def mbconv_chain(exp_block, dw_block, proj_block, x, residual=None, post_act=None):
     blocks = [b for b in (exp_block, dw_block, proj_block) if b is not None]
     if not isinstance(x, engine.NHWC) or not all(isinstance(b, ConvBlock) for b in blocks):
diff --git a/pytorchcv_amd/models/resnet.py b/pytorchcv_amd/models/resnet.py
--- a/pytorchcv_amd/models/resnet.py
+++ b/pytorchcv_amd/models/resnet.py
@@ -6,7 +6,7 @@
 import torch.nn as nn
 from .common.activ import lambda_relu
 from .common.norm import lambda_batchnorm2d
-from .common.conv import conv1x1_block, conv3x3_block, conv7x7_block, conv_block_pair, conv_block_maxpool
+from .common.conv import conv1x1_block, conv3x3_block, conv7x7_block, conv_block_pair, conv_block_maxpool, bottleneck_unit
 from ._tail import MaxPool2dNHWC, AvgPool2dNHWC, LinearHead, run_net, maybe_load_pretrained, init_conv_params, DEFAULT_ROOT
 from .. import engine
 
@@ -64,9 +64,22 @@
         identity = self.identity_conv(a) if self.resize_identity else a
         return self.body(a, residual=identity, post_act=self.activ)
 
+    def fused(self, a, check_only=False):
+        if self.resize_identity or not isinstance(self.body, ResBottleneck):
+            return None
+        b = self.body
+        return bottleneck_unit(b.conv1, b.conv2, b.conv3, a, self.activ, check_only=check_only)
+
     def run_chained(self, a, conv1_out=None, next_unit=None):
+        if conv1_out is None:
+            y = self.fused(a)
+            if y is not None:
+                return y, None
         body = self.body
         y = body.conv2(conv1_out if conv1_out is not None else body.conv1(a))
+        if isinstance(next_unit, ResUnit) and isinstance(y, engine.NHWC) and \
+                next_unit.fused(engine.ShapeOnly(y.N, y.H, y.W, body.conv3.conv.out_channels, y.dtype), check_only=True):
+            next_unit = None
         if next_unit is not None and self.resize_identity:
             pair = conv_block_pair(body.conv3, y, None, self.activ, next_unit.body.conv1, id_block=self.identity_conv, x0=a)
             if pair is not None:
```

New measurement: 90090 images/sec, median of 6. No clear change (+0.3%).
